# zzbuzzard/PATHS

Hardware: AMD Instinct MI355X
Metric: slides_per_sec_5level_K2048_D1024 (higher is better)
Workload: dtype f32 (products as 2 fp16 planes per operand = 22 bits, 3 fp16 MFMAs per block, fp32 accumulate); 1 GPU; 5-level PATHS recursion (forward, eval): K=2048 patches/level (level-0 grid 32x64, top_k 512, 10% background), D=1024 features, trans_dim 128 x 4 heads x 2 layers, LSTM ctx 256; 8 HBM-resident slides per GPU; slides_per_gpu=8, global_batch=8, levels=5, resident_batches_rotated=3, parallelism=slide-sharded x1 (no data-path collective)

## Files before the change

include/paths_hip.h:

```cpp
#ifndef PATHS_HIP_H
#define PATHS_HIP_H

#include <stddef.h>
#include <stdint.h>

#ifdef __cplusplus
extern "C" {
#endif

typedef void* paths_stream_t;

const char* paths_last_error(void);
const char* paths_build_info(void);
int paths_abi_version(void);

void* paths_event_create(void);
void* paths_stream_create_masked(const uint32_t* cu_mask, int words);
int paths_event_destroy(void* event);
int paths_stream_wait(paths_stream_t dst, paths_stream_t src, void* event);
int paths_set_stop_event(void* event);
int paths_flush_stop_event(paths_stream_t src);
int paths_stop_event_pending(void);
int paths_clear_stop_event(void);
int paths_record_event(void* event, paths_stream_t stream);
int paths_stream_wait_event(paths_stream_t dst, void* event);
int paths_memset_zero(void* p, size_t bytes, paths_stream_t stream);

int paths_lstm_cell(const float* x, int64_t ldx, const float* h0, int64_t ldh0, const float* c0, int64_t ldc0,
                    const float* w_gates, const float* b_gates, const float* w_mem, const float* b_mem,
                    float* state_out, int64_t ldso, float* y, int64_t ldy, float* ws_o, float* save_frm, float* save_tc,
                    const float* hp, const int* hp_row,
                    int M, int D, int Hc, const int64_t* num_ims, int rows_per_slide, int phases, paths_stream_t stream);

int paths_pe_table(const float* div_term, int pe_mode, int d, int rows, float* out, paths_stream_t stream);
int paths_importance_proj(const float* y, int64_t ldy, const float* w_ip, const float* b1, const float* w2, const float* b2 ,
                          const float* bp, const float* special, const float* div_term, const float* pe_table, int pe_rows,
                          const int64_t* locs,
                          const int64_t* num_ims, int rows_per_slide, int patch_size, int pe_mode, int imp_mul,
                          float* importance, float* tokens, float* save_hid, float* save_pproj, int M, int D, int Hi, int d,
                          int skip_padding, paths_stream_t stream);

int64_t paths_x6_packed_bytes(int Npad, int K, int planes);
int paths_x6_pack_weights(const float* w, int64_t ldw, void* out, int N, int Npad, int K, int planes, float w_scale,
                          paths_stream_t stream);
int paths_x6_pack_weights_t(const float* w, int64_t ldw, void* out, int N, int Npad, int K, int Kvalid, int planes, paths_stream_t stream);
int paths_lstm_cell_x6(const float* x, int64_t ldx, const int64_t* x_rows, const float* h0, int64_t ldh0, const float* c0, int64_t ldc0,
                       const void* w_gates_x6, const float* b_gates, const void* w_mem_x6, const float* b_mem,
                       float* state_out, int64_t ldso, float* y, int64_t ldy, float* ws_o, float* save_frm, float* save_tc,
                       const float* hp, const int* hp_row,
                       int M, int D, int Hc, const int64_t* num_ims, int rows_per_slide, int phases,
                       int planes, float wg_scale, float wm_scale, float a_scale, paths_stream_t stream);
int paths_lstm_cell_x6_h16(const float* x, int64_t ldx, const int64_t* x_rows, const float* h0, int64_t ldh0, const float* c0, int64_t ldc0,
                           const void* w_gates_x6, const float* b_gates, const void* w_mem_x6, const float* b_mem,
                           float* state_out, int64_t ldso, float* y, int64_t ldy, float* ws_o, float* save_frm, float* save_tc,
                           const float* hp, const int* hp_row,
                           int M, int D, int Hc, const int64_t* num_ims, int rows_per_slide, int phases,
                           int planes, float wg_scale, float wm_scale, float a_scale, paths_stream_t stream);
int paths_importance_proj_x6(const float* y, int64_t ldy, const int64_t* y_rows, const float* y_add, int64_t ldya, const void* w_ip_x6, const float* b1, const float* w2, const float* b2 ,
                             const float* bp, const float* special, const float* div_term, const float* pe_table, int pe_rows,
                             const int64_t* locs,
                             const int64_t* num_ims, int rows_per_slide, int patch_size, int pe_mode, int imp_mul,
                             float* importance, float* tokens, float* save_hid, float* save_pproj, int M, int D, int Hi, int d,
                             int skip_padding, int planes, float w_scale, float a_scale, float* splitk_ws, paths_stream_t stream);
int paths_importance_proj_x6_h16(const float* y, int64_t ldy, const int64_t* y_rows, const float* y_add, int64_t ldya, const void* w_ip_x6, const float* b1, const float* w2, const float* b2 ,
                                 const float* bp, const float* special, const float* div_term, const float* pe_table, int pe_rows,
                                 const int64_t* locs,
                                 const int64_t* num_ims, int rows_per_slide, int patch_size, int pe_mode, int imp_mul,
                                 float* importance, float* tokens, float* save_hid, float* save_pproj, int M, int D, int Hi, int d,
                                 int skip_padding, int planes, float w_scale, float a_scale, float* splitk_ws, paths_stream_t stream);
int64_t paths_importance_proj_x6_workspace(int M);
int paths_importance_qkv_x6(const float* y, int64_t ldy, const int64_t* y_rows, const float* y_add, int64_t ldya, const void* w_ip_x6,
                            const float* b1, const float* w2, const float* b2 , const float* bp, const float* special,
                            const float* pe_table, int pe_rows, const int64_t* locs, const int64_t* num_ims, int B, int N,
                            int patch_size, int pe_mode, int imp_mul, float* importance, float* tokens, int D, int skip_padding,
                            float w_scale, float a_scale, float* splitk_ws, const void* w_qkv, const float* bqkv, float s_wqkv,
                            float qscale, void* qkv_images, int phases, int alpha_from_importance, paths_stream_t stream);
int paths_importance_qkv_x6_h16(const float* y, int64_t ldy, const int64_t* y_rows, const float* y_add, int64_t ldya, const void* w_ip_x6,
                                const float* b1, const float* w2, const float* b2 , const float* bp, const float* special,
                                const float* pe_table, int pe_rows, const int64_t* locs, const int64_t* num_ims, int B, int N,
                                int patch_size, int pe_mode, int imp_mul, float* importance, float* tokens, int D, int skip_padding,
                                float w_scale, float a_scale, float* splitk_ws, const void* w_qkv, const float* bqkv, float s_wqkv,
                                float qscale, void* qkv_images, int phases, int alpha_from_importance, paths_stream_t stream);
int paths_gemm_nt_x6(const float* a, int64_t lda, const void* w_x6, int Kpacked, int k0, const float* b, float* out, int64_t ldo,
                     int M, int N, int Npad, int K, int act, const float* residual, int64_t ldr, const float* mask,
                     int64_t ldm, int accumulate, int planes, float w_scale, float a_scale, paths_stream_t stream);
int paths_gemm_add_nt_x6(const float* a, int64_t lda, const int64_t* a_rows, const float* a_add, int64_t ld_add, const void* w_x6, int Kpacked,
                         const float* b, float* out, int64_t ldo, int M, int N, int Npad, int K, int act, const int64_t* num_ims,
                         int rows_per_slide, float w_scale, float a_scale, paths_stream_t stream);
int paths_gemm_add_nt_x6_h16(const float* a, int64_t lda, const int64_t* a_rows, const float* a_add, int64_t ld_add, const void* w_x6, int Kpacked,
                             const float* b, float* out, int64_t ldo, int M, int N, int Npad, int K, int act, const int64_t* num_ims,
                             int rows_per_slide, float w_scale, float a_scale, paths_stream_t stream);
int paths_gemm_rows_nt_x6(const int64_t* a_rows, const void* w_x6, int Kpacked, int k0, float* out, int64_t ldo,
                          int M, int Npad, int K, int planes, float w_scale, float a_scale, paths_stream_t stream);

int paths_gemm_nt_f32(const float* a, int64_t lda, const float* w, int64_t ldw, const float* b, float* out, int64_t ldo,
                      int M, int N, int Npad, int K, int act, const float* residual, int64_t ldr, const float* mask,
                      int64_t ldm, int accumulate, paths_stream_t stream);
int64_t paths_gemm_tn_workspace(int N1, int N2, int splits);
int paths_gemm_tn_f32(const float* a, int64_t lda, const float* b0, int64_t ldb0, int nb0, const float* b1, int64_t ldb1,
                      float* out, int64_t ldo, int M, int N1, int N2, int splits, int accumulate, float* workspace,
                      paths_stream_t stream);
int paths_gemm_tn_x6(const float* a, int64_t lda, const float* b0, int64_t ldb0, int nb0, const float* b1, int64_t ldb1,
                     float* out, int64_t ldo, int M, int N1, int N2, int splits, int accumulate, float* workspace, int planes,
                     paths_stream_t stream);
int paths_colsum_f32(const float* a, int64_t lda, int M, int N, float* out, int splits, int accumulate, float* workspace,
                     paths_stream_t stream);
int paths_transpose_f32(const float* in, int64_t ldi, int R, int C, float* out, int64_t ldo, paths_stream_t stream);

int paths_adamw_chunk(void);
int paths_adamw_multi(const int64_t* table, const int64_t* numel, const int32_t* blocks, int nblocks, const float* step_size,
                      const float* bc2_sqrt, float wd_scale, int has_wd, float lerp_w, float beta2, float value, float eps, int flavor,
                      paths_stream_t stream);

int paths_lstm_bwd_a(const float* dh1, int64_t ldd, const float* dh1b, int64_t lddb, const float* o, const float* tc,
                     const int64_t* num_ims, int rows_per_slide, int64_t M, int D, float* dpre_o, int64_t ldo,
                     float* dpre_h, paths_stream_t stream);
int paths_lstm_bwd_b(const float* dc1_h, const float* dc1_ext, int64_t lde, const float* frm, const float* c0, int64_t ldc0,
                     const int64_t* num_ims, int rows_per_slide, int64_t M, int Hc, float* dg, int64_t ldg, float* dc0,
                     int64_t lddc0, paths_stream_t stream);
int paths_importance_bwd(const float* dtok, const float* pproj, const float* hid, const float* alpha, const float* w2,
                         const int64_t* num_ims, int rows_per_slide, int64_t M, int imp_mul, float* du, float* da, float* dah,
                         paths_stream_t stream);
int paths_layernorm_fwd_stats(const float* x, const float* add, const float* gamma, const float* beta, float* y, float* xhat,
                              float* rstd, int64_t rows, int d, float eps, paths_stream_t stream);
int paths_layernorm_bwd(const float* dy, const float* xhat, const float* rstd, const float* gamma, float* dx, float* dyxhat,
                        int64_t rows, int d, paths_stream_t stream);
int paths_layernorm_bwd_sums(const float* dy, const float* xhat, const float* rstd, const float* gamma, float* dx, float* slabs,
                             int64_t rows, int d, int rows_per_block, paths_stream_t stream);
int paths_reduce_slabs_f32(const float* slabs, int splits, int n, float* out, int accumulate, paths_stream_t stream);
int paths_defer_reductions(int on);
int paths_flush_reductions(int* n_entries, paths_stream_t stream);

int paths_attention_bwd_f32(const float* q, const float* k, const float* v, const float* o, const float* d_o, const float* lse,
                            const int64_t* num_ims, float* dqkv, float* ws_dsum, int B, int T, int H, int head_dim,
                            paths_stream_t stream);
int64_t paths_attention_token0_workspace(int B, int T, int H);
int paths_attention_token0_any(const float* qkv, int64_t ld, const int64_t* num_ims, float* a0, float* ws, int B, int T, int H, int head_dim,
                               float qscale, paths_stream_t stream);
int paths_attention_token0_fwd(const float* q, const float* k, const float* v, const int64_t* num_ims, float* a0, float* lse0, float* ws,
                               int B, int T, int H, int head_dim, uint64_t drop_key, float drop_p, paths_stream_t stream);
int paths_attention_token0_bwd(const float* q, const float* k, const float* v, const float* a0, const float* da0, const float* lse0,
                               const int64_t* num_ims, float* dqkv, float* ws, int B, int T, int H, int head_dim, uint64_t drop_key,
                               float drop_p, paths_stream_t stream);
int64_t paths_token0_attention_workspace(int B, int T, int d, int H);
int paths_token0_attention(const float* x, const int64_t* num_ims, const float* in_proj_weight, const float* in_proj_bias, float* attn_patch,
                           int64_t patch_ld, float* attn_self, int64_t self_ld, float* ws, int B, int T, int d, int H, int special_last,
                           paths_stream_t stream);
int64_t paths_attention_rollout_workspace(int B, int T, int d, int H);
int paths_attention_rollout_prepare(const float* x, const int64_t* num_ims, const float* in_proj_weight, const float* in_proj_bias, float* ws,
                                    int B, int T, int d, int H, int special_last, paths_stream_t stream);
int paths_attention_rollout_seed(const float* attn_patch, int64_t patch_ld, const float* attn_self, int64_t self_ld, const int64_t* num_ims,
                                 float* r, float* rollout, int64_t rollout_ld, float* rollout_self, int B, int T, int H, paths_stream_t stream);
int paths_attention_rollout_step(const float* ws, const int64_t* num_ims, const float* r_in, float* r_out, float* rollout, int64_t rollout_ld,
                                 float* rollout_self, int B, int T, int d, int H, paths_stream_t stream);

int paths_linear_f32(const float* a, int64_t lda, const float* w, const float* b, float* out, int64_t ldo,
                     int M, int N, int Npad, int K, int act, paths_stream_t stream);

int paths_attention_f32(const float* q, const float* k, const float* v, float* o, float* lse, const int64_t* num_ims,
                        int B, int T, int H, int head_dim, int max_queries, paths_stream_t stream);

int64_t paths_attention_x6_workspace(int B, int T, int H, int head_dim, int planes);
int paths_attention_x6(const float* q, const float* k, const float* v, float* o, float* lse, const int64_t* num_ims,
                       int B, int T, int H, int head_dim, int max_queries, void* workspace, int planes, int images_ready,
                       paths_stream_t stream);

int paths_token_layer_f32(const float* x_in, const float* attn, float* x_out,
                          const float* wo, const float* bo, const float* ln1g, const float* ln1b, const float* cab,
                          const float* ln2g, const float* ln2b, const float* w1, const float* b1, const float* w2,
                          const float* b2, const float* ln3g, const float* ln3b, const float* wqkv, const float* bqkv,
                          float* q, float* k, float* v, const int64_t* num_ims, int B, int T, int d, int H,
                          int do_post, int do_qkv, int skip_padding, float qscale, float eps, int max_tokens,
                          paths_stream_t stream);

int64_t paths_tlayer_h3_image_bytes(int part);
int paths_tlayer_pack_h3(int part, const float* wa, const float* wb, const float* wc, float s_a, float s_b, float s_c, void* out,
                         paths_stream_t stream);
int paths_token_layer_h3(const float* x_in, const float* attn, float* x_out, const void* w_post, const void* w_qkv,
                         const float* bo, const float* ln1g, const float* ln1b, const float* cab, const float* ln2g, const float* ln2b,
                         const float* b1, const float* b2, const float* ln3g, const float* ln3b, const float* bqkv,
                         float s_wo, float s_w1, float s_w2, float s_wqkv,
                         float* q, float* k, float* v, const int64_t* num_ims, int B, int T, int d, int H,
                         int do_post, int do_qkv, int skip_padding, float qscale, float eps, int max_tokens, void* qkv_images,
                         paths_stream_t stream);

int64_t paths_tlayer_ws_image_bytes(int part, int d);
int paths_tlayer_pack_ws(int part, const float* wa, const float* wb, const float* wc, float s_a, float s_b, float s_c, void* out, int d,
                         paths_stream_t stream);
int paths_token_layer_ws(const float* x_in, const float* attn, const void* attn_img, float* x_out, const void* w_post, const void* w_qkv,
                         const float* bo, const float* ln1g, const float* ln1b, const float* cab, const float* ln2g, const float* ln2b,
                         const float* b1, const float* b2, const float* ln3g, const float* ln3b, const float* bqkv,
                         float s_wo, float s_w1, float s_w2, float s_wqkv, void* qkv_images, const int64_t* num_ims,
                         int B, int T, int d, int H, int do_post, int do_qkv, int skip_padding, float qscale, float eps,
                         int* zero_words, int n_zero, paths_stream_t stream);
int paths_token_layer_ws_rows(const float* x_in, const float* attn, float* x_out, const void* w_post, const void* w_qkv,
                              const float* bo, const float* ln1g, const float* ln1b, const float* cab, const float* ln2g, const float* ln2b,
                              const float* b1, const float* b2, const float* ln3g, const float* ln3b, const float* bqkv,
                              float s_wo, float s_w1, float s_w2, float s_wqkv, float* qkv_rows, int64_t ld_qkv, const int64_t* num_ims,
                              int B, int T, int d, int do_post, int do_qkv, int skip_padding, float eps, paths_stream_t stream);
int paths_attention_h3_img(void* o_img, const int64_t* num_ims, int B, int T, int H, int head_dim, void* workspace, paths_stream_t stream);

int64_t paths_token0_ws_image_bytes(void);
int64_t paths_token0_ws_image_bytes_d(int d);
int64_t paths_token0_ws_partials(int B, int T);
int64_t paths_token0_ws_partials_d(int B, int T, int d);
int paths_token0_ws_supported(int B, int T, int d, int H);
int paths_token0_pack_ws(const float* wqkv, const float* bqkv, const float* wo, const float* bo, const float* w1, const float* w2, float qscale,
                         void* out, paths_stream_t stream);
int paths_token0_pack_ws_d(const float* wqkv, const float* bqkv, const float* wo, const float* bo, const float* w1, const float* w2, float qscale,
                           int d, void* out, paths_stream_t stream);
int paths_token0_tail_ws(const float* x1, const int64_t* num_ims, const void* img, const float* bv, const float* bo,
                         const float* ln1g, const float* ln1b, const float* cab, const float* ln2g, const float* ln2b,
                         const float* b1, const float* b2, const float* ln3g, const float* ln3b, const float* lnfg, const float* lnfb,
                         const float* ctx_prev, int64_t ctx_stride, const float* ctx_all, int ctx_depth,
                         const float* wcls, const float* bcls, int num_logits, int cls_in,
                         float* ctx_out, float* logits, float* partials, int* counters, int* status, int B, int T, int d, int H,
                         float eps, float eps_final, int special_last , paths_stream_t stream);

int paths_attention_any(const float* qkv, int64_t ld, float* o, const int64_t* num_ims, int B, int T, int H, int head_dim, float qscale,
                        int max_queries, paths_stream_t stream);
int64_t paths_attention_h3_any_workspace(int B, int T, int H, int head_dim);
int paths_attention_h3_any(const float* qkv, int64_t ld, float* o, const int64_t* num_ims, int B, int T, int H, int head_dim, float qscale,
                           void* workspace, paths_stream_t stream);
int paths_attention_h3_any_img(float* o, const int64_t* num_ims, int B, int T, int H, int head_dim, void* workspace, paths_stream_t stream);
int paths_layernorm_rows(const float* x, int64_t ldx, const float* add, const float* gamma, const float* beta, float* y, int64_t ldy,
                         int64_t rows, int d, float eps, paths_stream_t stream);
int paths_layernorm2_rows(const float* x, int64_t ldx, const float* g1, const float* b1, const float* add, const float* g2, const float* b2,
                          float* y, int64_t ldy, int64_t rows, int d, float eps, paths_stream_t stream);
int paths_importance_rows(const float* hid, int64_t ldh, const float* w2, const float* b2, const int64_t* num_ims, int rows_per_slide,
                          int64_t M, int Hi, float* importance, int relu , paths_stream_t stream);
int paths_tokens_assemble(const float* P, int64_t ldp, const float* importance, int imp_mul, const float* bp, const float* special,
                          const float* div_term, const int64_t* locs, int rows_per_slide, int patch_size, int pe_mode, int d, int B,
                          float* tokens, paths_stream_t stream);
int paths_importance_tokens_rows(const float* hid, int64_t ldh, const float* w2, const float* b2, const int64_t* num_ims, int rows_per_slide,
                                 int64_t M, int Hi, float* importance, int relu, int imp_mul, const float* bp, const float* special,
                                 const float* pe_table, int pe_rows, const int64_t* locs, int patch_size, int pe_mode, int d, float* tokens,
                                 paths_stream_t stream);
int paths_final_head_any(const float* x, int64_t slide_stride, const float* lng, const float* lnb, const float* ctx_prev, int64_t ctx_stride,
                         const float* ctx_all, int ctx_depth, const float* wcls, const float* bcls, int num_logits, int cls_in,
                         float* ctx_out, float* logits, int B, int d, float eps, paths_stream_t stream);

int paths_attention_any_train(const float* qkv, int64_t ld, float* o, float* lse, const int64_t* num_ims, int B, int T, int H, int head_dim,
                              float qscale, int max_queries, uint64_t drop_key, float drop_p, paths_stream_t stream);
int paths_attention_bwd_any(const float* qkv, int64_t ld, const float* o, const float* d_o, const float* lse, const int64_t* num_ims,
                            float* dqkv, float* ws_dsum, int B, int T, int H, int head_dim, float qscale, int max_queries,
                            uint64_t drop_key, float drop_p, paths_stream_t stream);
int paths_layernorm_fwd_stats_any(const float* x, const float* add, const float* gamma, const float* beta, float* y, float* xhat,
                                  float* rstd, int64_t rows, int d, float eps, paths_stream_t stream);
int paths_layernorm_bwd_any(const float* dy, const float* xhat, const float* rstd, const float* gamma, float* dx, float* dyxhat,
                            int64_t rows, int d, paths_stream_t stream);
int paths_layernorm_bwd_sums_any(const float* dy, const float* xhat, const float* rstd, const float* gamma, float* dx, float* slabs,
                                 int64_t rows, int d, int rows_per_block, paths_stream_t stream);
int paths_importance_rows_bwd_any(const float* dz_rows, const float* x, int D, const float* hid, const float* alpha, const float* w2,
                                  const int64_t* num_ims, int rows_per_slide, int64_t M, int Hi, float* dh, float* da, float* dah,
                                  paths_stream_t stream);
int paths_importance_bwd_any(const float* dtok, const float* pproj, const float* hid, const float* alpha, const float* w2,
                             const int64_t* num_ims, int rows_per_slide, int64_t M, int imp_mul, int Hi, int d, int64_t ldu, float* du,
                             float* da, float* dah, paths_stream_t stream);

int paths_token0_tail(const float* x_in, const float* q, const float* k, const float* v, const int64_t* num_ims,
                      const float* wo, const float* bo, const float* ln1g, const float* ln1b, const float* cab,
                      const float* ln2g, const float* ln2b, const float* w1, const float* b1, const float* w2,
                      const float* b2, const float* ln3g, const float* ln3b, const float* lnfg, const float* lnfb,
                      const float* ctx_prev, int64_t ctx_stride, const float* ctx_all, int ctx_depth,
                      const float* wcls, const float* bcls, int num_logits, int cls_in,
                      float* ctx_out, float* logits, float* ws_partials, int B, int T, int d, int H, float eps,
                      float eps_final, paths_stream_t stream);

int paths_final_head(const float* x, int64_t slide_stride, const float* lng, const float* lnb,
                     const float* ctx_prev, int64_t ctx_stride, const float* ctx_all, int ctx_depth,
                     const float* wcls, const float* bcls, int num_logits, int cls_in,
                     float* ctx_out, float* logits, int B, int d, float eps, paths_stream_t stream);

int paths_layernorm_f32(const float* x, const float* gamma, const float* beta, float* y, int64_t rows, int d,
                        float eps, paths_stream_t stream);

int paths_topk(const float* scores, int64_t ld, const int64_t* num_ims, int B, int n_max, int keep,
               int* keep_idx, int64_t ldk, int* keep_count, paths_stream_t stream);
int paths_topk_rows(const float* scores, int64_t ld, const int64_t* num_ims, int B, int n_max, int keep,
                    int* keep_idx, int64_t ldk, int* keep_count, const float* row_base, int64_t row_ld, int64_t slide_rows,
                    int64_t* kept_rows, const float* zero_row, paths_stream_t stream);

int paths_expand_children(const int* keep_idx, int64_t ldk, const int* keep_count, const int64_t* locs, int64_t n_cur,
                          int patch_size, const int* next_x, const int* next_y, const int64_t* mask_ptrs, int B,
                          int64_t n_next, int64_t* num_out, int64_t* locs_out, int64_t* parent_out, int* src_row,
                          int* src_cell, int* status, int* child_pos, int* hp_row, paths_stream_t stream);

int paths_candidate_children(const int* keep_idx, int64_t ldk, const int* keep_count, const int64_t* locs, int64_t n_cur,
                             int patch_size, const int* next_x, const int* next_y, int B, int* cand_count, int64_t* cand_cells,
                             int* cand_slot, paths_stream_t stream);
int paths_admit_children(const int* cand_count, const int64_t* cand_cells, const int* cand_slot, const uint8_t* cand_mask,
                         const int* keep_idx, int64_t ldk, const int* keep_count, int patch_size, int B, int64_t n_next,
                         int64_t* num_out, int64_t* locs_out, int64_t* parent_out, int* src_row, int* src_cell, int* status,
                         int* child_pos, int* hp_row, paths_stream_t stream);

int paths_fallback_all_cells(const int* next_x, const int* next_y, const int64_t* mask_ptrs, int patch_size, int B,
                             int64_t n_next, int64_t* num_out, int64_t* locs_out, int64_t* parent_out, int* src_row,
                             int* src_cell, int* status, int* hp_row, paths_stream_t stream);

int paths_gather_rows(const int64_t* grid_ptrs, const int* src_cell, int D, const float* state_cur, int64_t n_cur,
                      int64_t ld_state_cur, const int* src_row, int Dp, const int64_t* num_out, int B, int64_t n_next,
                      float* fts_out, float* state_out, int zero_pad, int64_t* row_ptrs, const float* zero_row,
                      paths_stream_t stream);
int paths_gather_rows_h16(const int64_t* grid_ptrs, const int* src_cell, int D, const float* state_cur, int64_t n_cur,
                          int64_t ld_state_cur, const int* src_row, int Dp, const int64_t* num_out, int B, int64_t n_next,
                          float* fts_out, float* state_out, int zero_pad, int64_t* row_ptrs, const float* zero_row,
                          paths_stream_t stream);

int paths_gather_kept_rows(const float* src, int64_t n_cur, int64_t ld_src, const int* keep_idx, int64_t ldk, const int* keep_count,
                           int D, int B, float* out, paths_stream_t stream);

int paths_gather_rows_bwd(const int* keep_idx, int64_t ldk, const int* keep_count, const int* child_pos, const float* d_next,
                          int64_t n_next, int Dp, float* d_cur, int64_t n_cur, int B, paths_stream_t stream);

int paths_sibling_sum(const int* keep_idx, int64_t ldk, const int* keep_count, const int* child_pos, const float* src, int64_t n_src,
                      int64_t ld_src, int width, float* dst, int64_t n_dst, int64_t ld_dst, int B, paths_stream_t stream);
int paths_scatter_kept_rows(const float* src, int64_t ldk, int64_t ld_src, const int* keep_idx, const int* keep_count, float* dst,
                            int64_t n_dst, int64_t ld_dst, int width, int B, paths_stream_t stream);

int paths_level0_batch(const int64_t* grid_ptrs, const int* gx, const int* gy, int B, int D, int patch_size, int64_t n0,
                       float* fts, int64_t* locs, int64_t* parent, int64_t* num_ims, int zero_pad, int64_t* row_ptrs,
                       const float* zero_row, paths_stream_t stream);
int paths_level0_batch_h16(const int64_t* grid_ptrs, const int* gx, const int* gy, int B, int D, int patch_size, int64_t n0,
                           float* fts, int64_t* locs, int64_t* parent, int64_t* num_ims, int zero_pad, int64_t* row_ptrs,
                           const float* zero_row, paths_stream_t stream);

int paths_stage_rows(int64_t* row_ptrs, int64_t rows, int row_bytes, void* stage, const void* zero_row, paths_stream_t stream);

int paths_saliency_rows(const float* dx, int64_t ldd, const float* x, int64_t ldx, const int64_t* num_ims, int rows_per_slide, int D,
                        int B, float* gxi, float* gnorm, paths_stream_t stream);

int paths_scale_add_rows(const float* x, const float* alpha, const float* h, const int64_t* num_ims, int rows_per_slide,
                         int D, int64_t M, int use_alpha, float* z, paths_stream_t stream);

int paths_tissue_mask(const float* grid, int64_t cells, int D, uint8_t* mask, paths_stream_t stream);

int paths_tissue_mask_absmax(const float* grid, int64_t cells, int D, uint8_t* mask, uint32_t* absmax_bits, paths_stream_t stream);
int paths_tissue_mask_absmax_h16(const void* grid, int64_t cells, int D, uint8_t* mask, uint32_t* absmax_bits, paths_stream_t stream);

int paths_synth_grid(float* grid, int X, int Y, int D, uint32_t slide_level_key, int level, uint64_t bg_threshold,
                     paths_stream_t stream);
int paths_synth_grid_h16(void* grid, int X, int Y, int D, uint32_t slide_level_key, int level, uint64_t bg_threshold,
                         paths_stream_t stream);

int paths_importance_rows_bwd(const float* dz_rows, const float* x, int D, const float* hid, const float* alpha, const float* w2,
                              const int64_t* num_ims, int rows_per_slide, int64_t M, float* dh, float* da, float* dah,
                              paths_stream_t stream);


int paths_dropout_rows(const float* x, int64_t ldx, const float* vec, const float* resid, int64_t ldr, float* out, int64_t ldo,
                       int64_t M, int N, uint64_t key, float p, paths_stream_t stream);
int paths_dropout_mask(float* mask, int64_t n, uint64_t key, float p, paths_stream_t stream);
int64_t paths_attention_fp8_workspace(int B, int T, int H, int head_dim);
int paths_attention_fp8(const float* q, const float* k, const float* v, float* o, const int64_t* num_ims, int B, int T, int H,
                        int head_dim, void* workspace, paths_stream_t stream);
int paths_attention_fp8_qkv(const float* qkv, int64_t ld, float* o, const int64_t* num_ims, int B, int T, int H, int head_dim, float qscale,
                            void* workspace, paths_stream_t stream);

int paths_fp8_scale(const float* x, int64_t ld, int64_t M, int K, float* scale, unsigned int* scratch, const int64_t* num_ims,
                    int rows_per_slide, paths_stream_t stream);
int paths_fp8_pack_weight(const float* w, int64_t ldw, int N, int K, uint8_t* w8, float* scale, unsigned int* scratch, paths_stream_t stream);
int paths_fp8_quantize(const float* x, int64_t ld, int M, int K, const float* scale, uint8_t* x8, paths_stream_t stream);
int paths_gemm_nt_fp8(const uint8_t* a8, const uint8_t* w8, const float* a_scale, const float* w_scale, const float* bias,
                      float* out, int64_t ldo, int M, int N, int K, int act, const float* residual, int64_t ldr, paths_stream_t stream);
int paths_gemm_nt_fp8_out8(const uint8_t* a8, const uint8_t* w8, const float* a_scale, const float* w_scale, const float* bias,
                           uint8_t* out8, const float* out_scale, unsigned int* out_absmax, int M, int N, int K, int act,
                           paths_stream_t stream);

int paths_attention_x6_dropout(const float* q, const float* k, const float* v, float* o, float* lse, const int64_t* num_ims, int B,
                               int T, int H, int head_dim, int max_queries, void* workspace, int planes, uint64_t drop_key,
                               float drop_p, paths_stream_t stream);
int paths_attention_bwd_f32_dropout(const float* q, const float* k, const float* v, const float* o, const float* d_o,
                                    const float* lse, const int64_t* num_ims, float* dqkv, float* ws_dsum, int B, int T, int H,
                                    int head_dim, uint64_t drop_key, float drop_p, paths_stream_t stream);
int64_t paths_attention_bwd_x6_workspace(int B, int T, int H, int head_dim);
int paths_attention_bwd_x6_dropout(const float* q, const float* k, const float* v, const float* o, const float* d_o, const float* lse,
                                   const int64_t* num_ims, float* dqkv, float* ws_dsum, void* images, int B, int T, int H, int head_dim,
                                   uint64_t drop_key, float drop_p, paths_stream_t stream);
int paths_attention_bwd_x6_planes(const float* q, const float* k, const float* v, const float* o, const float* d_o, const float* lse,
                                  const int64_t* num_ims, float* dqkv, float* ws_dsum, void* images, int B, int T, int H, int head_dim,
                                  uint64_t drop_key, float drop_p, int planes, paths_stream_t stream);

int64_t paths_attention_wide_workspace(int T, int head_dim);
int paths_attention_wide_fwd(const float* qkv, int64_t ld, float* o, float* lse, const int64_t* num_ims, int B, int T, int H, int head_dim,
                             float qscale, int max_queries, uint64_t drop_key, float drop_p, float* workspace, paths_stream_t stream);
int paths_attention_wide_bwd(const float* qkv, int64_t ld, const float* o, const float* d_o, const float* lse, const int64_t* num_ims,
                             float* dqkv, int B, int T, int H, int head_dim, float qscale, int max_queries, uint64_t drop_key, float drop_p,
                             float* workspace, paths_stream_t stream);

#ifdef __cplusplus
}
#endif
#endif
```

paths_amd/_lib.py:

```python
from __future__ import annotations

import ctypes as C
import os
from typing import Optional

import torch

_HERE = os.path.dirname(os.path.abspath(__file__))
LIB_PATH = os.environ.get("PATHS_HIP_LIB") or os.path.join(_HERE, "libpaths_hip.so")

_i64, _i32, _f32, _vp, _u32, _u64 = C.c_int64, C.c_int, C.c_float, C.c_void_p, C.c_uint32, C.c_uint64

SIGNATURES = {
    "paths_lstm_cell": [_vp, _i64, _vp, _i64, _vp, _i64, _vp, _vp, _vp, _vp, _vp, _i64, _vp, _i64, _vp, _vp, _vp, _vp, _vp,
                        _i32, _i32, _i32, _vp, _i32, _i32, _vp],
    "paths_pe_table": [_vp, _i32, _i32, _i32, _vp, _vp],
    "paths_importance_proj": [_vp, _i64, _vp, _vp, _vp, _vp, _vp, _vp, _vp, _vp, _i32, _vp, _vp, _i32, _i32, _i32, _i32,
                              _vp, _vp, _vp, _vp, _i32, _i32, _i32, _i32, _i32, _vp],
    "paths_gemm_nt_f32": [_vp, _i64, _vp, _i64, _vp, _vp, _i64, _i32, _i32, _i32, _i32, _i32, _vp, _i64, _vp, _i64, _i32, _vp],
    "paths_x6_pack_weights": [_vp, _i64, _vp, _i32, _i32, _i32, _i32, _f32, _vp],
    "paths_x6_pack_weights_t": [_vp, _i64, _vp, _i32, _i32, _i32, _i32, _i32, _vp],
    "paths_lstm_cell_x6": [_vp, _i64, _vp, _vp, _i64, _vp, _i64, _vp, _vp, _vp, _vp, _vp, _i64, _vp, _i64, _vp, _vp, _vp, _vp, _vp,
                           _i32, _i32, _i32, _vp, _i32, _i32, _i32, _f32, _f32, _f32, _vp],
    "paths_importance_proj_x6": [_vp, _i64, _vp, _vp, _i64, _vp, _vp, _vp, _vp, _vp, _vp, _vp, _vp, _i32, _vp, _vp, _i32, _i32, _i32, _i32,
                                 _vp, _vp, _vp, _vp, _i32, _i32, _i32, _i32, _i32, _i32, _f32, _f32, _vp, _vp],
    "paths_importance_qkv_x6": [_vp, _i64, _vp, _vp, _i64, _vp, _vp, _vp, _vp, _vp, _vp, _vp, _i32, _vp, _vp, _i32, _i32, _i32, _i32, _i32,
                                _vp, _vp, _i32, _i32, _f32, _f32, _vp, _vp, _vp, _f32, _f32, _vp, _i32, _i32, _vp],
    "paths_gemm_nt_x6": [_vp, _i64, _vp, _i32, _i32, _vp, _vp, _i64, _i32, _i32, _i32, _i32, _i32, _vp, _i64, _vp, _i64, _i32,
                         _i32, _f32, _f32, _vp],
    "paths_gemm_add_nt_x6": [_vp, _i64, _vp, _vp, _i64, _vp, _i32, _vp, _vp, _i64, _i32, _i32, _i32, _i32, _i32, _vp, _i32, _f32, _f32, _vp],
    "paths_gemm_tn_f32": [_vp, _i64, _vp, _i64, _i32, _vp, _i64, _vp, _i64, _i32, _i32, _i32, _i32, _i32, _vp, _vp],
    "paths_attention_fp8": [_vp, _vp, _vp, _vp, _vp, _i32, _i32, _i32, _i32, _vp, _vp],
    "paths_gemm_tn_x6": [_vp, _i64, _vp, _i64, _i32, _vp, _i64, _vp, _i64, _i32, _i32, _i32, _i32, _i32, _vp, _i32, _vp],
    "paths_colsum_f32": [_vp, _i64, _i32, _i32, _vp, _i32, _i32, _vp, _vp],
    "paths_transpose_f32": [_vp, _i64, _i32, _i32, _vp, _i64, _vp],
    "paths_attention_wide_fwd": [_vp, _i64, _vp, _vp, _vp, _i32, _i32, _i32, _i32, _f32, _i32, _u64, _f32, _vp, _vp],
    "paths_attention_wide_bwd": [_vp, _i64, _vp, _vp, _vp, _vp, _vp, _i32, _i32, _i32, _i32, _f32, _i32, _u64, _f32, _vp, _vp],
    "paths_sibling_sum": [_vp, _i64, _vp, _vp, _vp, _i64, _i64, _i32, _vp, _i64, _i64, _i32, _vp],
    "paths_scatter_kept_rows": [_vp, _i64, _i64, _vp, _vp, _vp, _i64, _i64, _i32, _i32, _vp],
    "paths_adamw_multi": [_vp, _vp, _vp, _i32, _vp, _vp, _f32, _i32, _f32, _f32, _f32, _f32, _i32, _vp],
    "paths_lstm_bwd_a": [_vp, _i64, _vp, _i64, _vp, _vp, _vp, _i32, _i64, _i32, _vp, _i64, _vp, _vp],
    "paths_lstm_bwd_b": [_vp, _vp, _i64, _vp, _vp, _i64, _vp, _i32, _i64, _i32, _vp, _i64, _vp, _i64, _vp],
    "paths_importance_bwd": [_vp, _vp, _vp, _vp, _vp, _vp, _i32, _i64, _i32, _vp, _vp, _vp, _vp],
    "paths_layernorm_fwd_stats": [_vp, _vp, _vp, _vp, _vp, _vp, _vp, _i64, _i32, _f32, _vp],
    "paths_attention_bwd_f32": [_vp, _vp, _vp, _vp, _vp, _vp, _vp, _vp, _vp, _i32, _i32, _i32, _i32, _vp],
    "paths_attention_token0_any": [_vp, _i64, _vp, _vp, _vp, _i32, _i32, _i32, _i32, _f32, _vp],
    "paths_attention_token0_fwd": [_vp, _vp, _vp, _vp, _vp, _vp, _vp, _i32, _i32, _i32, _i32, _u64, _f32, _vp],
    "paths_attention_token0_bwd": [_vp, _vp, _vp, _vp, _vp, _vp, _vp, _vp, _vp, _i32, _i32, _i32, _i32, _u64, _f32, _vp],
    "paths_token0_attention": [_vp, _vp, _vp, _vp, _vp, _i64, _vp, _i64, _vp, _i32, _i32, _i32, _i32, _i32, _vp],
    "paths_attention_rollout_prepare": [_vp, _vp, _vp, _vp, _vp, _i32, _i32, _i32, _i32, _i32, _vp],
    "paths_attention_rollout_seed": [_vp, _i64, _vp, _i64, _vp, _vp, _vp, _i64, _vp, _i32, _i32, _i32, _vp],
    "paths_attention_rollout_step": [_vp, _vp, _vp, _vp, _vp, _i64, _vp, _i32, _i32, _i32, _i32, _vp],
    "paths_layernorm_bwd": [_vp, _vp, _vp, _vp, _vp, _vp, _i64, _i32, _vp],
    "paths_layernorm_bwd_sums": [_vp, _vp, _vp, _vp, _vp, _vp, _i64, _i32, _i32, _vp],
    "paths_reduce_slabs_f32": [_vp, _i32, _i32, _vp, _i32, _vp],
    "paths_defer_reductions": [_i32],
    "paths_flush_reductions": [_vp, _vp],
    "paths_linear_f32": [_vp, _i64, _vp, _vp, _vp, _i64, _i32, _i32, _i32, _i32, _i32, _vp],
    "paths_attention_f32": [_vp, _vp, _vp, _vp, _vp, _vp, _i32, _i32, _i32, _i32, _i32, _vp],
    "paths_attention_x6": [_vp, _vp, _vp, _vp, _vp, _vp, _i32, _i32, _i32, _i32, _i32, _vp, _i32, _i32, _vp],
    "paths_tlayer_pack_h3": [_i32, _vp, _vp, _vp, _f32, _f32, _f32, _vp, _vp],
    "paths_token_layer_h3": [_vp] * 16 + [_f32, _f32, _f32, _f32, _vp, _vp, _vp, _vp, _i32, _i32, _i32, _i32, _i32, _i32, _i32, _f32, _f32, _i32, _vp, _vp],
    "paths_tlayer_pack_ws": [_i32, _vp, _vp, _vp, _f32, _f32, _f32, _vp, _i32, _vp],
    "paths_token_layer_ws": [_vp] * 17 + [_f32, _f32, _f32, _f32, _vp, _vp, _i32, _i32, _i32, _i32, _i32, _i32, _i32, _f32, _f32, _vp, _i32, _vp],
    "paths_token_layer_ws_rows": [_vp] * 16 + [_f32, _f32, _f32, _f32, _vp, _i64, _vp, _i32, _i32, _i32, _i32, _i32, _i32, _f32, _vp],
    "paths_token0_pack_ws": [_vp, _vp, _vp, _vp, _vp, _vp, _f32, _vp, _vp],
    "paths_token0_pack_ws_d": [_vp, _vp, _vp, _vp, _vp, _vp, _f32, _i32, _vp, _vp],
    "paths_token0_tail_ws": [_vp] * 16 + [_vp, _i64, _vp, _i32, _vp, _vp, _i32, _i32, _vp, _vp, _vp, _vp, _vp, _i32, _i32, _i32, _i32, _f32, _f32, _i32, _vp],
    "paths_attention_any": [_vp, _i64, _vp, _vp, _i32, _i32, _i32, _i32, _f32, _i32, _vp],
    "paths_attention_any_train": [_vp, _i64, _vp, _vp, _vp, _i32, _i32, _i32, _i32, _f32, _i32, _u64, _f32, _vp],
    "paths_layernorm_fwd_stats_any": [_vp, _vp, _vp, _vp, _vp, _vp, _vp, _i64, _i32, _f32, _vp],
    "paths_layernorm_bwd_any": [_vp, _vp, _vp, _vp, _vp, _vp, _i64, _i32, _vp],
    "paths_layernorm_bwd_sums_any": [_vp, _vp, _vp, _vp, _vp, _vp, _i64, _i32, _i32, _vp],
    "paths_importance_bwd_any": [_vp, _vp, _vp, _vp, _vp, _vp, _i32, _i64, _i32, _i32, _i32, _i64, _vp, _vp, _vp, _vp],
    "paths_importance_rows_bwd_any": [_vp, _vp, _i32, _vp, _vp, _vp, _vp, _i32, _i64, _i32, _vp, _vp, _vp, _vp],
    "paths_attention_bwd_any": [_vp, _i64, _vp, _vp, _vp, _vp, _vp, _vp, _i32, _i32, _i32, _i32, _f32, _i32, _u64, _f32, _vp],
    "paths_fp8_scale": [_vp, _i64, _i64, _i32, _vp, _vp, _vp, _i32, _vp],
    "paths_fp8_pack_weight": [_vp, _i64, _i32, _i32, _vp, _vp, _vp, _vp],
    "paths_fp8_quantize": [_vp, _i64, _i32, _i32, _vp, _vp, _vp],
    "paths_gemm_nt_fp8_out8": [_vp, _vp, _vp, _vp, _vp, _vp, _vp, _vp, _i32, _i32, _i32, _i32, _vp],
    "paths_gemm_nt_fp8": [_vp, _vp, _vp, _vp, _vp, _vp, _i64, _i32, _i32, _i32, _i32, _vp, _i64, _vp],
    "paths_attention_fp8_qkv": [_vp, _i64, _vp, _vp, _i32, _i32, _i32, _i32, _f32, _vp, _vp],
    "paths_attention_h3_any": [_vp, _i64, _vp, _vp, _i32, _i32, _i32, _i32, _f32, _vp, _vp],
    "paths_attention_h3_any_img": [_vp, _vp, _i32, _i32, _i32, _i32, _vp, _vp],
    "paths_layernorm_rows": [_vp, _i64, _vp, _vp, _vp, _vp, _i64, _i64, _i32, _f32, _vp],
    "paths_layernorm2_rows": [_vp, _i64, _vp, _vp, _vp, _vp, _vp, _vp, _i64, _i64, _i32, _f32, _vp],
    "paths_importance_rows": [_vp, _i64, _vp, _vp, _vp, _i32, _i64, _i32, _vp, _i32, _vp],
    "paths_importance_tokens_rows": [_vp, _i64, _vp, _vp, _vp, _i32, _i64, _i32, _vp, _i32, _i32, _vp, _vp, _vp, _i32, _vp, _i32, _i32, _i32, _vp, _vp],
    "paths_tokens_assemble": [_vp, _i64, _vp, _i32, _vp, _vp, _vp, _vp, _i32, _i32, _i32, _i32, _i32, _vp, _vp],
    "paths_final_head_any": [_vp, _i64, _vp, _vp, _vp, _i64, _vp, _i32, _vp, _vp, _i32, _i32, _vp, _vp, _i32, _i32, _f32, _vp],
    "paths_attention_h3_img": [_vp, _vp, _i32, _i32, _i32, _i32, _vp, _vp],
    "paths_token_layer_f32": [_vp] * 21 + [_vp, _i32, _i32, _i32, _i32, _i32, _i32, _i32, _f32, _f32, _i32, _vp],
    "paths_token0_tail": [_vp] * 20 + [_vp, _i64, _vp, _i32, _vp, _vp, _i32, _i32, _vp, _vp, _vp, _i32, _i32, _i32, _i32, _f32, _f32, _vp],
    "paths_final_head": [_vp, _i64, _vp, _vp, _vp, _i64, _vp, _i32, _vp, _vp, _i32, _i32, _vp, _vp, _i32, _i32, _f32, _vp],
    "paths_layernorm_f32": [_vp, _vp, _vp, _vp, _i64, _i32, _f32, _vp],
    "paths_topk": [_vp, _i64, _vp, _i32, _i32, _i32, _vp, _i64, _vp, _vp],
    "paths_topk_rows": [_vp, _i64, _vp, _i32, _i32, _i32, _vp, _i64, _vp, _vp, _i64, _i64, _vp, _vp, _vp],
    "paths_gemm_rows_nt_x6": [_vp, _vp, _i32, _i32, _vp, _i64, _i32, _i32, _i32, _i32, _f32, _f32, _vp],
    "paths_expand_children": [_vp, _i64, _vp, _vp, _i64, _i32, _vp, _vp, _vp, _i32, _i64, _vp, _vp, _vp, _vp, _vp, _vp, _vp, _vp, _vp],
    "paths_candidate_children": [_vp, _i64, _vp, _vp, _i64, _i32, _vp, _vp, _i32, _vp, _vp, _vp, _vp],
    "paths_admit_children": [_vp, _vp, _vp, _vp, _vp, _i64, _vp, _i32, _i32, _i64, _vp, _vp, _vp, _vp, _vp, _vp, _vp, _vp, _vp],
    "paths_gather_kept_rows": [_vp, _i64, _i64, _vp, _i64, _vp, _i32, _i32, _vp, _vp],
    "paths_gather_rows_bwd": [_vp, _i64, _vp, _vp, _vp, _i64, _i32, _vp, _i64, _i32, _vp],
    "paths_fallback_all_cells": [_vp, _vp, _vp, _i32, _i32, _i64, _vp, _vp, _vp, _vp, _vp, _vp, _vp, _vp],
    "paths_gather_rows": [_vp, _vp, _i32, _vp, _i64, _i64, _vp, _i32, _vp, _i32, _i64, _vp, _vp, _i32, _vp, _vp, _vp],
    "paths_level0_batch": [_vp, _vp, _vp, _i32, _i32, _i32, _i64, _vp, _vp, _vp, _vp, _i32, _vp, _vp, _vp],
    "paths_scale_add_rows": [_vp, _vp, _vp, _vp, _i32, _i32, _i64, _i32, _vp, _vp],
    "paths_importance_rows_bwd": [_vp, _vp, _i32, _vp, _vp, _vp, _vp, _i32, _i64, _vp, _vp, _vp, _vp],
    "paths_dropout_rows": [_vp, _i64, _vp, _vp, _i64, _vp, _i64, _i64, _i32, _u64, _f32, _vp],
    "paths_dropout_mask": [_vp, _i64, _u64, _f32, _vp],
    "paths_attention_x6_dropout": [_vp, _vp, _vp, _vp, _vp, _vp, _i32, _i32, _i32, _i32, _i32, _vp, _i32, _u64, _f32, _vp],
    "paths_attention_bwd_f32_dropout": [_vp, _vp, _vp, _vp, _vp, _vp, _vp, _vp, _vp, _i32, _i32, _i32, _i32, _u64, _f32, _vp],
    "paths_attention_bwd_x6_dropout": [_vp, _vp, _vp, _vp, _vp, _vp, _vp, _vp, _vp, _vp, _i32, _i32, _i32, _i32, _u64, _f32, _vp],
    "paths_attention_bwd_x6_planes": [_vp, _vp, _vp, _vp, _vp, _vp, _vp, _vp, _vp, _vp, _i32, _i32, _i32, _i32, _u64, _f32, _i32, _vp],
    "paths_stream_wait": [_vp, _vp, _vp],
    "paths_set_stop_event": [_vp],
    "paths_flush_stop_event": [_vp],
    "paths_stream_wait_event": [_vp, _vp],
    "paths_record_event": [_vp, _vp],
    "paths_event_destroy": [_vp],
    "paths_memset_zero": [_vp, C.c_size_t, _vp],
    "paths_tissue_mask": [_vp, _i64, _i32, _vp, _vp],
    "paths_tissue_mask_absmax": [_vp, _i64, _i32, _vp, _vp, _vp],
    "paths_synth_grid": [_vp, _i32, _i32, _i32, _u32, _i32, _u64, _vp],
    "paths_stage_rows": [_vp, _i64, _i32, _vp, _vp, _vp],
    "paths_saliency_rows": [_vp, _i64, _vp, _i64, _vp, _i32, _i32, _i32, _vp, _vp, _vp],
}
for _n in ("paths_lstm_cell_x6", "paths_importance_proj_x6", "paths_importance_qkv_x6", "paths_gemm_add_nt_x6", "paths_gather_rows",
           "paths_level0_batch", "paths_tissue_mask_absmax", "paths_synth_grid"):
    SIGNATURES[_n + "_h16"] = SIGNATURES[_n]
_PLAIN = {"paths_gemm_tn_workspace": (C.c_int64, [_i32, _i32, _i32]), "paths_x6_packed_bytes": (C.c_int64, [_i32, _i32, _i32]), "paths_tlayer_h3_image_bytes": (C.c_int64, [_i32]), "paths_tlayer_ws_image_bytes": (C.c_int64, [_i32, _i32]), "paths_token0_ws_image_bytes": (C.c_int64, []), "paths_token0_ws_partials": (C.c_int64, [_i32, _i32]), "paths_token0_ws_image_bytes_d": (C.c_int64, [_i32]), "paths_token0_ws_partials_d": (C.c_int64, [_i32, _i32, _i32]), "paths_token0_ws_supported": (_i32, [_i32, _i32, _i32, _i32]), "paths_attention_x6_workspace": (C.c_int64, [_i32, _i32, _i32, _i32, _i32]), "paths_attention_fp8_workspace": (C.c_int64, [_i32, _i32, _i32, _i32]), "paths_attention_bwd_x6_workspace": (C.c_int64, [_i32, _i32, _i32, _i32]), "paths_attention_token0_workspace": (C.c_int64, [_i32, _i32, _i32]), "paths_token0_attention_workspace": (C.c_int64, [_i32, _i32, _i32, _i32]), "paths_attention_rollout_workspace": (C.c_int64, [_i32, _i32, _i32, _i32]), "paths_attention_h3_any_workspace": (C.c_int64, [_i32, _i32, _i32, _i32]), "paths_importance_proj_x6_workspace": (C.c_int64, [_i32]), "paths_last_error": (C.c_char_p, []), "paths_build_info": (C.c_char_p, []), "paths_abi_version": (_i32, []), "paths_stop_event_pending": (_i32, []), "paths_clear_stop_event": (_i32, []), "paths_adamw_chunk": (_i32, []), "paths_attention_wide_workspace": (C.c_int64, [_i32, _i32]), "paths_event_create": (_vp, []), "paths_stream_create_masked": (_vp, [_vp, _i32])}

ABI_VERSION = 3
_lib: Optional[C.CDLL] = None


class PathsHipError(RuntimeError):
    pass


def load() -> C.CDLL:
    global _lib
    if _lib is None:
        if not os.path.isfile(LIB_PATH):
            raise PathsHipError(f"{LIB_PATH} not found: the HIP extension is not built (run __graft_entry__.build()); "
                                "paths_amd has no CPU fallback")
        lib = C.CDLL(LIB_PATH)
        lib.paths_abi_version.restype = _i32
        if lib.paths_abi_version() != ABI_VERSION:
            raise PathsHipError(f"{LIB_PATH} has ABI version {lib.paths_abi_version()}, this binding needs {ABI_VERSION}: rebuild it "
                                "(__graft_entry__.build())")
        for name, args in SIGNATURES.items():
            fn = getattr(lib, name)
            fn.argtypes, fn.restype = args, _i32
        for name, (res, args) in _PLAIN.items():
            fn = getattr(lib, name)
            fn.argtypes, fn.restype = args, res
        _lib = lib
    return _lib


def ptr(t):
    if t is None or type(t) is int:
        return t
    return t.data_ptr()


_RAW_STREAM = getattr(torch._C, "_cuda_getCurrentRawStream", None)
_GET_DEVICE = getattr(torch._C, "_cuda_getDevice", None)


def stream() -> int:
    if _RAW_STREAM is not None and _GET_DEVICE is not None:
        return _RAW_STREAM(_GET_DEVICE())
    return torch.cuda.current_stream().cuda_stream


TAPE = None
TAPE_EVENTS = None


def call(name: str, *args):
    lib = load()
    fn = getattr(lib, name)
    rc = fn(*args)
    if rc != 0:
        raise PathsHipError(f"{name} failed ({rc}): {lib.paths_last_error().decode()}")
    if TAPE is not None:
        TAPE.append((fn, args, name))
        fb = fork_behind.active
        if fb is not None and fb.taken_at is None and name != "paths_set_stop_event" and not lib.paths_stop_event_pending():
            fb.taken_at = len(TAPE) - 1


def stream_wait(dst: "torch.cuda.Stream", src: "torch.cuda.Stream"):
    dst.wait_stream(src)
    if TAPE is not None:
        lib = load()
        pool = TAPE_EVENTS if TAPE_EVENTS is not None else [[], 0]
        if pool[1] == len(pool[0]):
            ev = lib.paths_event_create()
            if not ev:
                raise PathsHipError("paths_event_create failed")
            pool[0].append(ev)
        ev = pool[0][pool[1]]
        pool[1] += 1
        TAPE.append((lib.paths_stream_wait, (dst.cuda_stream, src.cuda_stream, ev), "paths_stream_wait"))


STOP_EVENTS = __import__("os").environ.get("PATHS_STOP_EVENTS", "1") != "0"


_TAPE_PLUMBING = {"paths_set_stop_event", "paths_flush_stop_event", "paths_stream_wait_event", "paths_stream_wait", "paths_record_event",
                  "paths_clear_stop_event"}


class fork_behind:

    active = None

    def __init__(self, dsts, src):
        self.dsts, self.src = list(dsts), src
        self.ev = None
        self.taken_at = None

    def __enter__(self):
        if TAPE is not None and STOP_EVENTS:
            lib = load()
            pool = TAPE_EVENTS if TAPE_EVENTS is not None else [[], 0]
            if pool[1] == len(pool[0]):
                e = lib.paths_event_create()
                if not e:
                    raise PathsHipError("paths_event_create failed")
                pool[0].append(e)
            self.ev = pool[0][pool[1]]
            pool[1] += 1
            call("paths_set_stop_event", self.ev)
            self.prev, fork_behind.active = fork_behind.active, self
        return self

    def __exit__(self, et, ev, tb):
        if self.ev is not None:
            fork_behind.active = self.prev
            if et is not None:
                load().paths_clear_stop_event()
                return False
            call("paths_flush_stop_event", self.src.cuda_stream)
            if self.taken_at is not None and any(nm not in _TAPE_PLUMBING for _, _, nm in TAPE[self.taken_at + 1:]):
                call("paths_record_event", self.ev, self.src.cuda_stream)
            for d in self.dsts:
                call("paths_stream_wait_event", d.cuda_stream, self.ev)
        elif et is None:
            for d in self.dsts:
                stream_wait(d, self.src)
        return False


def zeros(shape, **kw) -> torch.Tensor:
    t = torch.zeros(shape, **kw)
    if TAPE is not None:
        TAPE.append((load().paths_memset_zero, (t.data_ptr(), t.numel() * t.element_size(), stream()), "paths_memset_zero"))
    return t


def require_cuda(*tensors: torch.Tensor):
    for t in tensors:
        if t is not None and not t.is_cuda:
            raise PathsHipError("paths_amd runs on the GPU only: got a CPU tensor (no CPU fallback)")


def float_from_bits(bits: int) -> float:
    import struct
    bits &= 0xFFFFFFFF
    return float("inf") if bits >= 0x7F800000 else struct.unpack("<f", struct.pack("<I", bits))[0]


def absmax(t: torch.Tensor) -> float:
    require_cuda(t)
    assert t.dtype == torch.float32 and t.is_contiguous() and t.numel() % 4 == 0
    bits = torch.zeros((1,), dtype=torch.int32, device=t.device)
    D = t.shape[-1] if (t.dim() > 1 and t.shape[-1] % 4 == 0) else 4
    call("paths_tissue_mask_absmax", t.data_ptr(), t.numel() // D, D, None, bits.data_ptr(), stream())
    return float_from_bits(int(bits.item()))
```

paths_amd/csrc/gemm_x6.hip:

```cpp
#include "common.h"
#include "gemm_epi.h"
#include "finish_qkv.h"
#include "split.h"

#ifndef PATHS_X6_PART
#define PATHS_X6_PART 0
#endif

namespace {
using namespace paths_epi;

constexpr int FRAG = 1024;
template <int NP> constexpr int planes_of() { return NP == 4 ? 2 : NP; }
template <int NP> constexpr int subt() { return planes_of<NP>() * FRAG; }

struct X6Operands {
  const float* A0; int64_t lda0; int K0;
  const int64_t* A0rows;
  const float* A1; int64_t lda1; int K1;
  const float* Aadd; int64_t ldadd;
  const char* Wt;
  int64_t w_group_stride;
  int M;
  const int64_t* num_ims;
  int rows_per_slide;
  float a_scale;
  int ksplit = 1;
};

template <int NP, int WTM, int WTN, int PF, bool ADD, bool ROWS, class Epi, int OCC = 1, bool A16 = false>
__global__ void __launch_bounds__(256) __attribute__((amdgpu_waves_per_eu(OCC, OCC)))
gemm_x6_kernel(X6Operands g, Epi epi) {
  static_assert(NP == 2 || NP == 3 || NP == 4, "two fp16 planes, three bf16 planes or two bf16 planes");
  static_assert(!A16 || (NP == 2 && ROWS), "fp16 A rows: two-plane fp16 split, row-pointer form");
  constexpr int PL = planes_of<NP>();
  constexpr bool A1P = A16 && !ADD;
  constexpr int PLA = A1P ? 1 : PL;
  constexpr int SUBT = subt<NP>();
  constexpr int SUBTA = PLA * FRAG;
  constexpr int NPROD = NP == 3 ? 6 : A1P ? 2 : 3;
  constexpr int BM = WTM * 64, BN = WTN * 64;
  constexpr int SA = 2 * WTM, SB = 2 * WTN;
  constexpr int STAGE = SA * SUBTA + SB * SUBT;
  constexpr int NA = BM / 64;
  constexpr int NPB = SB * PL, NB = (NPB + 3) / 4;
  static_assert(WTM % 2 == 0, "A fragment register slots alternate per accumulator row");
  extern __shared__ __attribute__((aligned(16))) char smem[];
  const int tid = threadIdx.x, lane = tid & 63, wave = __builtin_amdgcn_readfirstlane(tid >> 6), wm = wave >> 1, wn = wave & 1;

  const int nbx = gridDim.x, nby = gridDim.y, nblk = nbx * nby;
  const int lin = xcd_tile_order(blockIdx.y * nbx + blockIdx.x, nblk);
  constexpr int GM = 8;
  const int per_group = GM * nbx;
  const int grp = lin / per_group, in_grp = lin - grp * per_group;
  const int rows_in_grp = min(GM, nby - grp * GM);
  const int by = grp * GM + in_grp % rows_in_grp, bx = in_grp / rows_in_grp;
  const int m0 = by * BM, n0 = bx * BN;
  if (block_all_padding(g.num_ims, g.rows_per_slide, m0, BM, g.M)) return;

  const int arow = tid >> 2, ac = tid & 3;
  uint32_t aoff0[NA], aoff1[NA], aoffs[ADD ? NA : 1]; int awr[NA];
  typedef const f32x4 __attribute__((address_space(1))) * gptr_f4;
  typedef const u32x2 __attribute__((address_space(1))) * gptr_h4;
  gptr_f4 rowp[ROWS && !A16 ? NA : 1];
  gptr_h4 rowh[A16 ? NA : 1];
#pragma unroll
  for (int p = 0; p < NA; ++p) {
    const int row = p * 64 + arow;
    const int64_t grow = min(m0 + row, g.M - 1);
    aoff0[p] = ROWS ? 0u : (uint32_t)((grow * g.lda0 + 4 * ac) * 4);
    if constexpr (A16) rowh[p] = reinterpret_cast<gptr_h4>(static_cast<uintptr_t>(g.A0rows[grow]) + 8 * ac);
    else if constexpr (ROWS) rowp[p] = reinterpret_cast<gptr_f4>(static_cast<uintptr_t>(g.A0rows[grow]) + 16 * ac);
    aoff1[p] = (uint32_t)((grow * g.lda1 + 4 * ac) * 4);
    if constexpr (ADD) aoffs[p] = (uint32_t)((grow * g.ldadd + 4 * ac) * 4);
    awr[p] = (row >> 5) * SUBTA + (ac >> 1) * 512 + (row & 31) * 16 + (ac & 1) * 8;
  }
  const int K0w = g.ksplit > 1 ? g.K0 / g.ksplit : g.K0;
  const int kofs = g.ksplit > 1 ? (int)blockIdx.z * K0w : 0;
  if (kofs != 0) {
#pragma unroll
    for (int p = 0; p < NA; ++p) {
      aoff0[p] += (uint32_t)kofs * 4u;
      if constexpr (A16) rowh[p] += kofs >> 2;
      else if constexpr (ROWS) rowp[p] += kofs >> 2;
      if constexpr (ADD) aoffs[p] += (uint32_t)kofs * 4u;
    }
  }
  const int nk0 = K0w >> 4, nk = (K0w + g.K1) >> 4;
  const char* bbase[NB]; int bwr[NB];
#pragma unroll
  for (int i = 0; i < NB; ++i) {
    int pc = wave + 4 * i;
    if (pc >= NPB) pc -= 4;
    const int sub = pc / PL, pl = pc % PL;
    bbase[i] = g.Wt + ((int64_t)(n0 >> 5) + sub) * g.w_group_stride + pl * FRAG;
    bwr[i] = (A1P ? SA * SUBTA + sub * SUBT : (SA + sub) * SUBT) + pl * FRAG + lane * 16;
  }
  static_assert(PF == 1 || PF == 2, "one or two register sets");
  f32x4 sa[PF][NA], sadd[ADD ? PF : 1][ADD ? NA : 1]; u32x4 sbr[PF][NB];
  u32x2 sh[A16 ? PF : 1][A16 ? NA : 1];
  uint32_t hi[NA][2], mid[NP != 2 ? NA : 1][2], lo[NA][2];
  float* const anyA = const_cast<float*>(ROWS ? reinterpret_cast<const float*>(g.Wt) : g.A0);
  const auto rsA0 = __builtin_amdgcn_make_buffer_rsrc(anyA, 0, 0xFFFFFFFFu, 0x00020000);
  const auto rsA1 = __builtin_amdgcn_make_buffer_rsrc(g.A1 ? const_cast<float*>(g.A1) : anyA, 0, 0xFFFFFFFFu, 0x00020000);
  const auto rsAdd = __builtin_amdgcn_make_buffer_rsrc(ADD ? const_cast<float*>(g.Aadd) : anyA, 0, 0xFFFFFFFFu, 0x00020000);
  const auto rsW = __builtin_amdgcn_make_buffer_rsrc(const_cast<char*>(g.Wt), 0, 0xFFFFFFFFu, 0x00020000);
  const int lane16 = lane * 16;
  int bsoff[NB];
#pragma unroll
  for (int i = 0; i < NB; ++i) bsoff[i] = (int)(bbase[i] - g.Wt) + (kofs >> 4) * SUBT;
  auto gload_a = [&](int set, int q, int kt) {
    const bool first = kt < nk0;
    const int soff = (first ? kt : kt - nk0) * 64;
    if constexpr (A16) {
      sh[set][q] = rowh[q][kt * 4];
    } else if constexpr (ROWS) {
      sa[set][q] = rowp[q][kt * 4];
    } else {
      const u32x4 raw = first ? __builtin_amdgcn_raw_buffer_load_b128(rsA0, (int)aoff0[q], soff, 0)
                              : __builtin_amdgcn_raw_buffer_load_b128(rsA1, (int)aoff1[q], soff, 0);
      sa[set][q] = __builtin_bit_cast(f32x4, raw);
    }
    if constexpr (ADD) {
      sadd[set][q] = __builtin_bit_cast(f32x4, __builtin_amdgcn_raw_buffer_load_b128(rsAdd, (int)aoffs[q], kt * 64, 0));
    }
  };
  auto gload_b = [&](int set, int q, int kt) {
    sbr[set][q] = __builtin_amdgcn_raw_buffer_load_b128(rsW, lane16, bsoff[q] + kt * SUBT, 0);
  };
  constexpr int PRE = ADD ? (A16 ? 2 : 1) : 0;
  constexpr int NS = A1P ? 2 : (NP == 3 ? 12 : NP == 4 ? 7 : 5) + PRE;
  float tf[NA][2];
  const uint32_t s2 = A1P ? __builtin_bit_cast(uint32_t, f16x2{(_Float16)g.a_scale, (_Float16)g.a_scale}) : 0u;
  auto a_step = [&](int set, int q, int st0, int buf) __attribute__((always_inline)) {
    f32x4& v = sa[set][q];
    const int st = st0 - PRE;
    if constexpr (ADD && A16) {
      if (st0 == 0) { v[0] = h_lo(sh[set][q][0]) + sadd[set][q][0]; v[1] = h_hi(sh[set][q][0]) + sadd[set][q][1]; }
      if (st0 == 1) { v[2] = h_lo(sh[set][q][1]) + sadd[set][q][2]; v[3] = h_hi(sh[set][q][1]) + sadd[set][q][3]; }
    } else if constexpr (ADD) {
      if (st0 == 0) v += sadd[set][q];
    }
    if constexpr (A1P) {
      if (st == 0) {
        asm("v_pk_mul_f16 %0, %1, %2" : "=v"(hi[q][0]) : "v"(sh[set][q][0]), "v"(s2));
        asm("v_pk_mul_f16 %0, %1, %2" : "=v"(hi[q][1]) : "v"(sh[set][q][1]), "v"(s2));
      }
      if (st == 1) *reinterpret_cast<u32x2*>(smem + buf * STAGE + awr[q]) = u32x2{hi[q][0], hi[q][1]};
    } else if constexpr (NP == 3) {
      if (st == 0) { hi[q][0] = pk_bf16(v[0], v[1]); hi[q][1] = pk_bf16(v[2], v[3]); }
      if (st == 1) { tf[q][0] = bf_lo(hi[q][0]); tf[q][1] = bf_hi(hi[q][0]); }
      if (st == 2) { v[0] -= tf[q][0]; v[1] -= tf[q][1]; }
      if (st == 3) { tf[q][0] = bf_lo(hi[q][1]); tf[q][1] = bf_hi(hi[q][1]); }
      if (st == 4) { v[2] -= tf[q][0]; v[3] -= tf[q][1]; }
      if (st == 5) { mid[q][0] = pk_bf16(v[0], v[1]); mid[q][1] = pk_bf16(v[2], v[3]); }
      if (st == 6) { tf[q][0] = bf_lo(mid[q][0]); tf[q][1] = bf_hi(mid[q][0]); }
      if (st == 7) { v[0] -= tf[q][0]; v[1] -= tf[q][1]; }
      if (st == 8) { tf[q][0] = bf_lo(mid[q][1]); tf[q][1] = bf_hi(mid[q][1]); }
      if (st == 9) { v[2] -= tf[q][0]; v[3] -= tf[q][1]; }
      if (st == 10) { lo[q][0] = pk_bf16(v[0], v[1]); lo[q][1] = pk_bf16(v[2], v[3]); }
      if (st == 11) {
        char* d = smem + buf * STAGE + awr[q];
        *reinterpret_cast<u32x2*>(d) = u32x2{hi[q][0], hi[q][1]};
        *reinterpret_cast<u32x2*>(d + FRAG) = u32x2{mid[q][0], mid[q][1]};
        *reinterpret_cast<u32x2*>(d + 2 * FRAG) = u32x2{lo[q][0], lo[q][1]};
      }
    } else if constexpr (NP == 4) {
      if (st == 0) { hi[q][0] = pk_bf16(v[0], v[1]); hi[q][1] = pk_bf16(v[2], v[3]); }
      if (st == 1) { tf[q][0] = bf_lo(hi[q][0]); tf[q][1] = bf_hi(hi[q][0]); }
      if (st == 2) { v[0] -= tf[q][0]; v[1] -= tf[q][1]; }
      if (st == 3) { tf[q][0] = bf_lo(hi[q][1]); tf[q][1] = bf_hi(hi[q][1]); }
      if (st == 4) { v[2] -= tf[q][0]; v[3] -= tf[q][1]; }
      if (st == 5) { mid[q][0] = pk_bf16(v[0], v[1]); mid[q][1] = pk_bf16(v[2], v[3]); }
      if (st == 6) {
        char* d = smem + buf * STAGE + awr[q];
        *reinterpret_cast<u32x2*>(d) = u32x2{hi[q][0], hi[q][1]};
        *reinterpret_cast<u32x2*>(d + FRAG) = u32x2{mid[q][0], mid[q][1]};
      }
    } else {
      if (st == 0) v *= g.a_scale;
      if (st == 1) { hi[q][0] = pk_f16(v[0], v[1]); hi[q][1] = pk_f16(v[2], v[3]); }
      if (st == 2) {
        asm("v_fma_mixlo_f16 %0, %1, -1.0, %2 op_sel_hi:[1,0,0]" : "=v"(lo[q][0]) : "v"(hi[q][0]), "v"(v[0]));
        asm("v_fma_mixlo_f16 %0, %1, -1.0, %2 op_sel_hi:[1,0,0]" : "=v"(lo[q][1]) : "v"(hi[q][1]), "v"(v[2]));
      }
      if (st == 3) {
        asm("v_fma_mixhi_f16 %0, %1, -1.0, %2 op_sel:[1,0,0] op_sel_hi:[1,0,0]" : "+v"(lo[q][0]) : "v"(hi[q][0]), "v"(v[1]));
        asm("v_fma_mixhi_f16 %0, %1, -1.0, %2 op_sel:[1,0,0] op_sel_hi:[1,0,0]" : "+v"(lo[q][1]) : "v"(hi[q][1]), "v"(v[3]));
      }
      if (st == 4) {
        char* d = smem + buf * STAGE + awr[q];
        *reinterpret_cast<u32x2*>(d) = u32x2{hi[q][0], hi[q][1]};
        *reinterpret_cast<u32x2*>(d + FRAG) = u32x2{lo[q][0], lo[q][1]};
      }
    }
  };
  auto swrite_b = [&](int set, int q, int buf) { *reinterpret_cast<u32x4*>(smem + buf * STAGE + bwr[q]) = sbr[set][q]; };

  f32x16 acc[WTM][WTN];
  epi.template init<WTM, WTN>(acc, m0 + wm * WTM * 32, n0 + wn * WTN * 32, lane, g.M);

  const char* sA = smem + (wm * WTM) * SUBTA + lane * 16;
  const char* sB = A1P ? smem + SA * SUBTA + (wn * WTN) * SUBT + lane * 16 : smem + (SA + wn * WTN) * SUBT + lane * 16;
  u32x4 fa[2][PLA], fb[2][WTN][PL];
  auto read_a = [&](int buf, int i, int slot, int p) { fa[slot][p] = *reinterpret_cast<const u32x4*>(sA + buf * STAGE + i * SUBTA + p * FRAG); };
  auto read_b = [&](int buf, int j, int slot, int p) { fb[slot][j][p] = *reinterpret_cast<const u32x4*>(sB + buf * STAGE + j * SUBT + p * FRAG); };
  constexpr int RG = WTN * NPROD;
  auto one_mfma = [&](int gq, int sb) __attribute__((always_inline)) {
    const int i = gq / RG, j = (gq % RG) / NPROD, t = gq % NPROD, sl = i & 1;
    if constexpr (NP == 3) {
      constexpr int PA_[6] = {2, 0, 1, 1, 0, 0}, PB_[6] = {0, 2, 1, 0, 1, 0};
      acc[i][j] = __builtin_amdgcn_mfma_f32_32x32x16_bf16(__builtin_bit_cast(bf16x8, fa[sl][PA_[t]]), __builtin_bit_cast(bf16x8, fb[sb][j][PB_[t]]), acc[i][j], 0, 0, 0);
    } else if constexpr (NP == 4) {
      constexpr int PA_[3] = {1, 0, 0}, PB_[3] = {0, 1, 0};
      acc[i][j] = __builtin_amdgcn_mfma_f32_32x32x16_bf16(__builtin_bit_cast(bf16x8, fa[sl][PA_[t]]), __builtin_bit_cast(bf16x8, fb[sb][j][PB_[t]]), acc[i][j], 0, 0, 0);
    } else if constexpr (A1P) {
      constexpr int PB_[2] = {1, 0};
      acc[i][j] = __builtin_amdgcn_mfma_f32_32x32x16_f16(__builtin_bit_cast(f16x8, fa[sl][0]), __builtin_bit_cast(f16x8, fb[sb][j][PB_[t]]), acc[i][j], 0, 0, 0);
    } else {
      constexpr int PA_[3] = {1, 0, 0}, PB_[3] = {0, 1, 0};
      acc[i][j] = __builtin_amdgcn_mfma_f32_32x32x16_f16(__builtin_bit_cast(f16x8, fa[sl][PA_[t]]), __builtin_bit_cast(f16x8, fb[sb][j][PB_[t]]), acc[i][j], 0, 0, 0);
    }
  };
  constexpr int AG = (WTM - 1) * RG;
  constexpr auto fits = [](int spg) constexpr {
    return PF == 1 ? ((NS + spg - 1) / spg) * NA + NB <= AG : (NS * NA + spg - 1) / spg + NB <= AG;
  };
  constexpr int SPG = fits(1) ? 1 : fits(2) ? 2 : fits(3) ? 3 : 4;
  static_assert(fits(SPG), "staging does not fit before the barrier");
  constexpr int GPC = (NS + SPG - 1) / SPG;
  constexpr int GA2 = (NS * NA + SPG - 1) / SPG;
  constexpr int TS = PF == 1 ? GPC * NA + NB : GA2 + NB + NA + NB;
  static_assert(TS <= WTM * RG, "staging does not fit in a stage");
  constexpr int AR0 = RG / 2;
  auto staging_slot = [&](auto sc, int kt, auto bufc, auto m1c, auto m2c) __attribute__((always_inline)) {
    constexpr int s = decltype(sc)::value, buf = decltype(bufc)::value;
    constexpr bool more1 = decltype(m1c)::value, more2 = decltype(m2c)::value;
    constexpr int set = PF == 2 ? (buf ^ 1) : 0;
    if constexpr (PF == 1) {
      if constexpr (s < GPC * NA) {
        constexpr int q = s / GPC, g0 = s % GPC;
        if constexpr (more1) {
          static_for<g0 * SPG, (g0 + 1) * SPG < NS ? (g0 + 1) * SPG : NS>([&](auto mc) __attribute__((always_inline)) {
            a_step(set, q, decltype(mc)::value, buf ^ 1);
          });
        }
        if constexpr (more2 && g0 == GPC - 1) gload_a(set, q, kt + 1 + PF);
      } else if constexpr (s < TS) {
        if constexpr (more1) swrite_b(set, s - GPC * NA, buf ^ 1);
        if constexpr (more2) gload_b(set, s - GPC * NA, kt + 1 + PF);
      }
    } else {
      if constexpr (s < GA2) {
        if constexpr (more1) {
          static_for<s * SPG, (s + 1) * SPG < NS * NA ? (s + 1) * SPG : NS * NA>([&](auto mc) __attribute__((always_inline)) {
            constexpr int m = decltype(mc)::value;
            a_step(set, m / NS, m % NS, buf ^ 1);
          });
        }
      } else if constexpr (s < GA2 + NB) {
        if constexpr (more1) swrite_b(set, s - GA2, buf ^ 1);
      } else if constexpr (s < GA2 + NB + NA) {
        if constexpr (more2) gload_a(set, s - GA2 - NB, kt + 1 + PF);
      } else if constexpr (s < TS) {
        if constexpr (more2) gload_b(set, s - GA2 - NB - NA, kt + 1 + PF);
      }
    }
  };
  auto stage_body = [&](int kt, auto bufc, auto m1c, auto m2c) __attribute__((always_inline)) {
    constexpr int buf = decltype(bufc)::value, sb = buf;
    constexpr bool more1 = decltype(m1c)::value, more2 = decltype(m2c)::value;
    constexpr int set = PF == 2 ? (buf ^ 1) : 0;
    static_for<0, AG>([&](auto gc) __attribute__((always_inline)) {
      constexpr int gq = decltype(gc)::value, i = gq / RG, gr = gq % RG;
      one_mfma(gq, sb);
      if constexpr (gr >= AR0 && gr < AR0 + PLA) read_a(buf, i + 1, (i + 1) & 1, gr - AR0);
      staging_slot(std::integral_constant<int, gq>{}, kt, bufc, m1c, m2c);
      __builtin_amdgcn_sched_barrier(0);
    });
    __syncthreads();
    __builtin_amdgcn_sched_barrier(0);
    static_for<AG, WTM * RG>([&](auto gc) __attribute__((always_inline)) {
      constexpr int gq = decltype(gc)::value, gr = gq % RG;
      one_mfma(gq, sb);
      if constexpr (more1) {
        static_for<2 * gr, 2 * gr + 2>([&](auto fc) __attribute__((always_inline)) {
          constexpr int f = decltype(fc)::value;
          if constexpr (f < PLA) read_a(buf ^ 1, 0, 0, f);
          else if constexpr (f < PLA + PL * WTN) read_b(buf ^ 1, (f - PLA) / PL, sb ^ 1, (f - PLA) % PL);
        });
      }
      staging_slot(std::integral_constant<int, gq>{}, kt, bufc, m1c, m2c);
      __builtin_amdgcn_sched_barrier(0);
    });
  };
  constexpr std::integral_constant<int, 0> I0{};
  constexpr std::integral_constant<int, 1> I1{};
  constexpr std::true_type T{};
  constexpr std::false_type F{};

#pragma unroll
  for (int q = 0; q < NA; ++q) gload_a(0, q, 0);
#pragma unroll
  for (int q = 0; q < NB; ++q) gload_b(0, q, 0);
#pragma unroll
  for (int q = 0; q < NA; ++q)
#pragma unroll
    for (int st = 0; st < NS; ++st) a_step(0, q, st, 0);
#pragma unroll
  for (int q = 0; q < NB; ++q) swrite_b(0, q, 0);
#pragma unroll
  for (int sidx = 1; sidx <= PF; ++sidx) {
#pragma unroll
    for (int q = 0; q < NA; ++q) gload_a(PF == 2 ? (sidx & 1) : 0, q, sidx);
#pragma unroll
    for (int q = 0; q < NB; ++q) gload_b(PF == 2 ? (sidx & 1) : 0, q, sidx);
  }
  __syncthreads();
#pragma unroll
  for (int p = 0; p < PLA; ++p) read_a(0, 0, 0, p);
#pragma unroll
  for (int j = 0; j < WTN; ++j)
#pragma unroll
    for (int p = 0; p < PL; ++p) read_b(0, j, 0, p);
  for (int kt = 0; kt < nk - 2 * PF; kt += 2) {
    __builtin_amdgcn_sched_barrier(0);
    stage_body(kt, I0, T, T);
    stage_body(kt + 1, I1, T, T);
  }
  if constexpr (PF == 2) {
    stage_body(nk - 4, I0, T, T);
    stage_body(nk - 3, I1, T, F);
  }
  stage_body(nk - 2, I0, T, F);
  stage_body(nk - 1, I1, F, F);
  __syncthreads();
  epi.template run<WTM, WTN, 2, 2>(acc, m0 + wm * WTM * 32, n0 + wn * WTN * 32, lane, wm, wn, g.M, reinterpret_cast<float*>(smem));
}

template <int NP>
__global__ void x6_pack_kernel(const float* __restrict__ w, int64_t ldw, uint16_t* __restrict__ out, int N, int Npad, int K, float wscale) {
  const int64_t i = blockIdx.x * (int64_t)blockDim.x + threadIdx.x;
  if (i >= (int64_t)Npad * K) return;
  const int n = (int)(i / K), k = (int)(i % K);
  const float v = n < N ? w[(int64_t)n * ldw + k] * wscale : 0.f;
  uint16_t* o = out + ((int64_t)(n >> 5) * (K >> 4) + (k >> 4)) * (subt<NP>() / 2) + ((k >> 3) & 1) * 256 + (n & 31) * 8 + (k & 7);
  if constexpr (NP == 3) {
    const __bf16 h = (__bf16)v; const float r1 = v - (float)h;
    const __bf16 m = (__bf16)r1; const float r2 = r1 - (float)m;
    const __bf16 l = (__bf16)r2;
    o[0] = __builtin_bit_cast(uint16_t, h); o[FRAG / 2] = __builtin_bit_cast(uint16_t, m); o[FRAG] = __builtin_bit_cast(uint16_t, l);
  } else if constexpr (NP == 4) {
    const __bf16 h = (__bf16)v; const float r1 = v - (float)h;
    const __bf16 m = (__bf16)r1;
    o[0] = __builtin_bit_cast(uint16_t, h); o[FRAG / 2] = __builtin_bit_cast(uint16_t, m);
  } else {
    const _Float16 h = (_Float16)v; const float r1 = v - (float)h;
    const _Float16 l = (_Float16)r1;
    o[0] = __builtin_bit_cast(uint16_t, h); o[FRAG / 2] = __builtin_bit_cast(uint16_t, l);
  }
}

template <int NP>
__global__ void x6_pack_t_kernel(const float* __restrict__ w, int64_t ldw, uint16_t* __restrict__ out, int N, int Npad, int K, int Kvalid) {
  static_assert(NP == 3 || NP == 4, "bf16 planes (scale 1)");
  const int64_t i = blockIdx.x * (int64_t)blockDim.x + threadIdx.x;
  if (i >= (int64_t)Npad * (K >> 3)) return;
  const int n = (int)(i % Npad), k0 = (int)(i / Npad) * 8;
  uint16_t h[8], m[8], l[8];
#pragma unroll
  for (int j = 0; j < 8; ++j) {
    const int k = k0 + j;
    const float v = (n < N && k < Kvalid) ? w[(int64_t)k * ldw + n] : 0.f;
    const __bf16 hh = (__bf16)v; const float r1 = v - (float)hh;
    const __bf16 mm = (__bf16)r1; const float r2 = r1 - (float)mm;
    const __bf16 ll = (__bf16)r2;
    h[j] = __builtin_bit_cast(uint16_t, hh); m[j] = __builtin_bit_cast(uint16_t, mm); l[j] = __builtin_bit_cast(uint16_t, ll);
  }
  uint16_t* o = out + ((int64_t)(n >> 5) * (K >> 4) + (k0 >> 4)) * (subt<NP>() / 2) + ((k0 >> 3) & 1) * 256 + (n & 31) * 8;
  typedef uint16_t u16x8 __attribute__((ext_vector_type(8)));
  *reinterpret_cast<u16x8*>(o) = u16x8{h[0], h[1], h[2], h[3], h[4], h[5], h[6], h[7]};
  *reinterpret_cast<u16x8*>(o + FRAG / 2) = u16x8{m[0], m[1], m[2], m[3], m[4], m[5], m[6], m[7]};
  if constexpr (NP == 3) *reinterpret_cast<u16x8*>(o + FRAG) = u16x8{l[0], l[1], l[2], l[3], l[4], l[5], l[6], l[7]};
}

template <int NP, int WTM, int WTN, int PF, bool ADD, bool ROWS, class Epi, int OCC = 1, bool A16 = false>
int launch_x6_np(const X6Operands& g, int Npad, const Epi& epi, hipStream_t stream, const char* name) {
  constexpr int BM = WTM * 64, BN = WTN * 64;
  constexpr size_t lds = 2ull * (2 * WTM * ((A16 && !ADD) ? FRAG : subt<NP>()) + 2 * WTN * subt<NP>());
  const int K = g.K0 + g.K1;
  PATHS_REQUIRE(g.M > 0, "%s: M must be > 0", name);
  PATHS_REQUIRE(g.K0 > 0 && g.K0 % 16 == 0 && g.K1 % 16 == 0 && K % 32 == 0 && K >= 128, "%s: K panels (%d,%d): multiples of 16, total a multiple of 32, >= 128", name, g.K0, g.K1);
  PATHS_REQUIRE(Npad % BN == 0, "%s: packed N (%d) must be a multiple of %d", name, Npad, BN);
  PATHS_REQUIRE(g.lda0 % 4 == 0 && g.lda1 % 4 == 0, "%s: leading dims must be multiples of 4 floats", name);
  PATHS_REQUIRE(((uintptr_t)g.A0 % 16 == 0) && ((uintptr_t)g.A1 % 16 == 0) && ((uintptr_t)g.Wt % 16 == 0), "%s: operands must be 16-byte aligned", name);
  PATHS_REQUIRE(ROWS == (g.A0rows != nullptr) && (!ROWS || g.K1 == 0), "%s: row-pointer form is single-panel", name);
  PATHS_REQUIRE((int64_t)g.M * (g.lda0 > g.lda1 ? (g.lda0 > g.ldadd ? g.lda0 : g.ldadd) : (g.lda1 > g.ldadd ? g.lda1 : g.ldadd)) * 4 < (int64_t)1 << 32, "%s: A panel larger than 4 GiB", name);
  auto kern = gemm_x6_kernel<NP, WTM, WTN, PF, ADD, ROWS, Epi, OCC, A16>;
  PATHS_LDS_OPT_IN(kern, lds, name);
  PATHS_REQUIRE(g.ksplit == 1 || (g.ksplit > 1 && g.K1 == 0 && g.K0 % (32 * g.ksplit) == 0 && g.K0 / g.ksplit >= 128), "%s: split-K needs a single panel and k windows that are multiples of 32, >= 128", name);
  dim3 grid(Npad / BN, (g.M + BM - 1) / BM, g.ksplit);
  hipLaunchKernelGGL(kern, grid, dim3(256), lds, stream, g, epi);
  PATHS_LAUNCH_CHECK(name);
  return PATHS_OK;
}

struct EpiRaw {
  float* ws; int64_t zstride; int ntn;
  template <int WTM, int WTN>
  __device__ __forceinline__ void init(f32x16 (&acc)[WTM][WTN], int, int, int, int) const {
#pragma unroll
    for (int i = 0; i < WTM; ++i)
#pragma unroll
      for (int j = 0; j < WTN; ++j)
#pragma unroll
        for (int r = 0; r < 16; ++r) acc[i][j][r] = 0.f;
  }
  template <int WTM, int WTN, int WGM, int WGN>
  __device__ __forceinline__ void run(f32x16 (&acc)[WTM][WTN], int row0, int col0, int lane, int, int, int, float*) const {
    float* base = ws + (int64_t)blockIdx.z * zstride;
#pragma unroll
    for (int i = 0; i < WTM; ++i)
#pragma unroll
      for (int j = 0; j < WTN; ++j) {
        f32x4* t = reinterpret_cast<f32x4*>(base + ((int64_t)((row0 >> 5) + i) * ntn + (col0 >> 5) + j) * 1024) + lane;
#pragma unroll
        for (int q = 0; q < 4; ++q) {
          const f32x4 v = f32x4{acc[i][j][4 * q], acc[i][j][4 * q + 1], acc[i][j][4 * q + 2], acc[i][j][4 * q + 3]};
          t[64 * q] = v;
        }
      }
  }
};

template <int NZ, class Epi>
__global__ void __launch_bounds__(256)
x6_finish_kernel(const float* __restrict__ ws, int64_t zstride, int ntn, int M, const int64_t* __restrict__ num_ims, int rows_per_slide, Epi epi) {
  extern __shared__ __attribute__((aligned(16))) char smem[];
  const int tid = threadIdx.x, lane = tid & 63, wave = __builtin_amdgcn_readfirstlane(tid >> 6), wm = wave >> 1, wn = wave & 1;
  const int m0 = blockIdx.x * 64;
  if (block_all_padding(num_ims, rows_per_slide, m0, 64, M)) return;
  const int row0 = m0 + wm * 32, col0 = wn * 128;
  f32x16 acc[1][4];
#pragma unroll
  for (int j = 0; j < 4; ++j) {
    const f32x4* t = reinterpret_cast<const f32x4*>(ws + ((int64_t)(row0 >> 5) * ntn + (col0 >> 5) + j) * 1024) + lane;
#pragma unroll
    for (int q = 0; q < 4; ++q) {
      f32x4 v = t[64 * q];
#pragma unroll
      for (int z = 1; z < NZ; ++z) v += *reinterpret_cast<const f32x4*>(reinterpret_cast<const float*>(t + 64 * q) + z * zstride);
      acc[0][j][4 * q] = v[0]; acc[0][j][4 * q + 1] = v[1]; acc[0][j][4 * q + 2] = v[2]; acc[0][j][4 * q + 3] = v[3];
    }
  }
  epi.template run<1, 4, 2, 2>(acc, row0, col0, lane, wm, wn, M, reinterpret_cast<float*>(smem));
}

template <int WTM, int WTN, int PF, bool ADD, class Epi>
int launch_x6(int planes, const X6Operands& g, int Npad, const Epi& epi, hipStream_t stream, const char* name) {
  if (g.A0rows != nullptr) {
    if (planes == 2) return launch_x6_np<2, WTM, WTN, PF, ADD, true>(g, Npad, epi, stream, name);
    return paths_set_error(PATHS_EUNSUPPORTED, "%s: row pointers need planes = 2", name);
  }
  if constexpr (std::is_same<Epi, EpiBias>::value && !ADD) {
    if (planes == 4) return launch_x6_np<4, WTM, WTN, PF, ADD, false>(g, Npad, epi, stream, name);
  }
  if (planes == 3) return launch_x6_np<3, WTM, WTN, PF, ADD, false>(g, Npad, epi, stream, name);
  if (planes == 2) return launch_x6_np<2, WTM, WTN, PF, ADD, false>(g, Npad, epi, stream, name);
  return paths_set_error(PATHS_EINVAL, "%s: planes must be 3 (bf16 x6) or 2 (fp16 x3), got %d", name, planes);
}

constexpr int H_OCC = 3;
constexpr int H_TRAIN_OCC = 2;

inline int plane_count(int planes) { return planes == 4 ? 2 : planes; }
inline int64_t group_stride(int planes, int Kpacked) { return (int64_t)(Kpacked / 16) * plane_count(planes) * FRAG; }
inline bool pow2(float x) { int e; return x > 0.f && frexpf(x, &e) == 0.5f; }
inline bool h16_scale_ok(float a_scale) { return pow2(a_scale) && a_scale >= 1.0f && a_scale <= 32768.0f; }

}

extern "C" {

#if PATHS_X6_PART == 0 || PATHS_X6_PART == 1
int64_t paths_x6_packed_bytes(int Npad, int K, int planes) { return (int64_t)Npad * K * 2 * plane_count(planes); }

int paths_x6_pack_weights(const float* w, int64_t ldw, void* out, int N, int Npad, int K, int planes, float w_scale, hipStream_t stream) {
  PATHS_REQUIRE(N > 0 && Npad >= N && Npad % 32 == 0 && K % 16 == 0, "x6_pack_weights: bad shape N=%d Npad=%d K=%d", N, Npad, K);
  PATHS_REQUIRE((uintptr_t)out % 16 == 0, "x6_pack_weights: out must be 16-byte aligned");
  PATHS_REQUIRE(((planes == 3 || planes == 4) && w_scale == 1.0f) || (planes == 2 && pow2(w_scale)), "x6_pack_weights: planes 3 / 4 (bf16) with w_scale 1, or planes 2 with a power-of-two w_scale");
  const int64_t n = (int64_t)Npad * K;
  const dim3 grid((unsigned)((n + 255) / 256));
  if (planes == 4) hipLaunchKernelGGL(x6_pack_kernel<4>, grid, dim3(256), 0, stream, w, ldw, reinterpret_cast<uint16_t*>(out), N, Npad, K, 1.0f);
  else if (planes == 3) hipLaunchKernelGGL(x6_pack_kernel<3>, grid, dim3(256), 0, stream, w, ldw, reinterpret_cast<uint16_t*>(out), N, Npad, K, 1.0f);
  else hipLaunchKernelGGL(x6_pack_kernel<2>, grid, dim3(256), 0, stream, w, ldw, reinterpret_cast<uint16_t*>(out), N, Npad, K, w_scale);
  PATHS_LAUNCH_CHECK("x6_pack_weights");
  return PATHS_OK;
}

int paths_x6_pack_weights_t(const float* w, int64_t ldw, void* out, int N, int Npad, int K, int Kvalid, int planes, hipStream_t stream) {
  PATHS_REQUIRE(N > 0 && Npad >= N && Npad % 32 == 0 && K % 16 == 0 && Kvalid > 0 && Kvalid <= K, "x6_pack_weights_t: bad shape N=%d Npad=%d K=%d Kvalid=%d", N, Npad, K, Kvalid);
  PATHS_REQUIRE(w != nullptr && out != nullptr && (uintptr_t)out % 16 == 0, "x6_pack_weights_t: null / unaligned operand");
  PATHS_REQUIRE(planes == 3 || planes == 4, "x6_pack_weights_t: planes 3 or 4 (bf16)");
  const int64_t n = (int64_t)Npad * (K / 8);
  const dim3 grid((unsigned)((n + 255) / 256));
  if (planes == 4) hipLaunchKernelGGL(x6_pack_t_kernel<4>, grid, dim3(256), 0, stream, w, ldw, reinterpret_cast<uint16_t*>(out), N, Npad, K, Kvalid);
  else hipLaunchKernelGGL(x6_pack_t_kernel<3>, grid, dim3(256), 0, stream, w, ldw, reinterpret_cast<uint16_t*>(out), N, Npad, K, Kvalid);
  PATHS_LAUNCH_CHECK("x6_pack_weights_t");
  return PATHS_OK;
}

}
namespace {
template <bool A16>
int lstm_cell_x6(const float* x, int64_t ldx, const int64_t* x_rows, const float* h0, int64_t ldh0, const float* c0, int64_t ldc0,
                 const void* w_gates_x6, const float* b_gates, const void* w_mem_x6, const float* b_mem,
                 float* state_out, int64_t ldso, float* y, int64_t ldy, float* ws_o, float* save_frm, float* save_tc,
                 const float* hp, const int* hp_row, int M, int D, int Hc, const int64_t* num_ims, int rows_per_slide,
                 int phases, int planes, float wg_scale, float wm_scale, float a_scale, hipStream_t stream) {
  PATHS_REQUIRE(D % 256 == 0 && Hc % 64 == 0, "lstm_cell_x6: D (%d) must be a multiple of 256 and Hc (%d) of 64", D, Hc);
  if constexpr (A16) {
    PATHS_REQUIRE(x_rows != nullptr && x == nullptr && planes == 2, "lstm_cell_x6_h16: fp16 rows are given as x_rows (planes = 2)");
    PATHS_REQUIRE(h16_scale_ok(a_scale), "lstm_cell_x6_h16: a_scale must be a power of two in [1, 2^15]");
  }
  PATHS_REQUIRE(hp != nullptr || (h0 == nullptr) == (c0 == nullptr), "lstm_cell_x6: h0 and c0 must both be given or both be null");
  PATHS_REQUIRE((hp == nullptr) == (hp_row == nullptr) && (hp == nullptr || h0 == nullptr),
                "lstm_cell_x6: hp/hp_row come together and replace h0 (the h half of the gate GEMM was done per parent)");
  PATHS_REQUIRE(planes == 3 || (pow2(wg_scale) && pow2(wm_scale) && pow2(a_scale)), "lstm_cell_x6: scales must be powers of two");
  PATHS_REQUIRE(x_rows == nullptr || (h0 == nullptr && y == nullptr && save_tc == nullptr), "lstm_cell_x6: x_rows (rows addressed in place) excludes h0, y and the training saves");
  if (planes == 3) wg_scale = wm_scale = a_scale = 1.0f;
  const char* wg = reinterpret_cast<const char*>(w_gates_x6);
  const int64_t gs = group_stride(planes, 2 * D);
  const float sg = 1.0f / (wg_scale * a_scale), sm = 1.0f / (wm_scale * a_scale);
  X6Operands g{x, ldx, D, x_rows, h0, h0 ? ldh0 : 0, h0 ? D : 0, nullptr, 0, wg, gs, M, num_ims, rows_per_slide, a_scale};
  const bool small_m = planes == 2 && M <= 8192 && (h0 == nullptr);
  if (phases & 1) {
    EpiLstmC e{b_gates, c0, ldc0, state_out + D, ldso, save_frm, (int64_t)3 * Hc, hp, (int64_t)3 * Hc + D, hp_row, sg};
    int rc;
    if constexpr (A16) {
      rc = small_m ? launch_x6_np<2, 2, 3, 2, false, true, decltype(e), 1, true>(g, 3 * Hc, e, stream, "lstm_cell_x6_h16(c, 128-row tiles)")
                   : launch_x6_np<2, 4, 3, 1, false, true, decltype(e), 1, true>(g, 3 * Hc, e, stream, "lstm_cell_x6_h16(c)");
    } else if (small_m) rc = x_rows ? launch_x6_np<2, 2, 3, 2, false, true>(g, 3 * Hc, e, stream, "lstm_cell_x6(c, 128-row tiles)")
                             : launch_x6_np<2, 2, 3, 2, false, false>(g, 3 * Hc, e, stream, "lstm_cell_x6(c, 128-row tiles)");
    else rc = launch_x6<4, 3, 1, false>(planes, g, 3 * Hc, e, stream, "lstm_cell_x6(c)");
    if (rc) return rc;
  }
  const bool o_raw = y == nullptr && save_tc == nullptr && save_frm == nullptr;
  if (phases & 2) {
    X6Operands go = g;
    go.Wt = wg + (int64_t)(3 * Hc / 32) * gs;
    int rc;
    if (o_raw) {
      EpiLstmORaw e{b_gates + 3 * Hc, ws_o, D, D, hp, (int64_t)3 * Hc + D, hp_row, 3 * Hc, sg};
      if constexpr (A16) {
        rc = small_m ? launch_x6_np<2, 2, 4, 2, false, true, decltype(e), 1, true>(go, D, e, stream, "lstm_cell_x6_h16(o, raw, 128-row tiles)")
                     : launch_x6_np<2, 4, 4, 1, false, true, decltype(e), 1, true>(go, D, e, stream, "lstm_cell_x6_h16(o, raw)");
      } else if (small_m) rc = x_rows ? launch_x6_np<2, 2, 4, 2, false, true>(go, D, e, stream, "lstm_cell_x6(o, raw, 128-row tiles)")
                               : launch_x6_np<2, 2, 4, 2, false, false>(go, D, e, stream, "lstm_cell_x6(o, raw, 128-row tiles)");
      else rc = launch_x6<4, 4, 1, false>(planes, go, D, e, stream, "lstm_cell_x6(o, raw)");
    } else {
      EpiLstmO e{b_gates + 3 * Hc, ws_o, D, D, hp, (int64_t)3 * Hc + D, hp_row, 3 * Hc, sg};
      if constexpr (A16) rc = launch_x6_np<2, 4, 4, 1, false, true, decltype(e), 1, true>(go, D, e, stream, "lstm_cell_x6_h16(o)");
      else rc = launch_x6<4, 4, 1, false>(planes, go, D, e, stream, "lstm_cell_x6(o)");
    }
    if (rc) return rc;
  }
  if (phases & 4) {
    X6Operands gh{state_out + D, ldso, Hc, nullptr, nullptr, 0, 0, nullptr, 0, reinterpret_cast<const char*>(w_mem_x6), group_stride(planes, Hc), M, num_ims, rows_per_slide, a_scale};
    int rc;
    PATHS_REQUIRE(save_tc == nullptr || y != nullptr, "lstm_cell_x6: save_tc (training) needs y");
    PATHS_REQUIRE(planes == 2 || planes == 3, "lstm_cell_x6: planes must be 3 (bf16 x6) or 2 (fp16 x3), got %d", planes);
    if (save_tc != nullptr) {
      EpiLstmH<true, true> e{b_mem, ws_o, D, x, ldx, state_out, ldso, y, ldy, D, save_tc, sm};
      if (planes == 2) rc = launch_x6_np<2, 2, 2, 2, false, false, decltype(e), H_TRAIN_OCC>(gh, D, e, stream, "lstm_cell_x6(h, save, 128x128)");
      else rc = launch_x6_np<3, 4, 4, 1, false, false>(gh, D, e, stream, "lstm_cell_x6(h, save)");
    } else if (y != nullptr) {
      EpiLstmH<true, false> e{b_mem, ws_o, D, x, ldx, state_out, ldso, y, ldy, D, nullptr, sm};
      rc = launch_x6<4, 4, 1, false>(planes, gh, D, e, stream, "lstm_cell_x6(h)");
    } else if (o_raw) {
      EpiLstmH<false, false, true> e{b_mem, ws_o, D, x, ldx, state_out, ldso, nullptr, 0, D, nullptr, sm};
      if (planes == 2) rc = launch_x6_np<2, 2, 2, 2, false, false, decltype(e), H_OCC>(gh, D, e, stream, "lstm_cell_x6(h, raw o, 128x128)");
      else rc = launch_x6_np<3, 4, 4, 1, false, false>(gh, D, e, stream, "lstm_cell_x6(h, raw o)");
    } else {
      EpiLstmH<false, false> e{b_mem, ws_o, D, x, ldx, state_out, ldso, nullptr, 0, D, nullptr, sm};
      if (planes == 2) rc = launch_x6_np<2, 2, 2, 2, false, false, decltype(e), H_OCC>(gh, D, e, stream, "lstm_cell_x6(h, no y, 128x128)");
      else rc = launch_x6_np<3, 4, 4, 1, false, false>(gh, D, e, stream, "lstm_cell_x6(h, no y)");
    }
    if (rc) return rc;
  }
  return PATHS_OK;
}
}
extern "C" {

int paths_lstm_cell_x6(const float* x, int64_t ldx, const int64_t* x_rows, const float* h0, int64_t ldh0, const float* c0, int64_t ldc0,
                       const void* w_gates_x6, const float* b_gates, const void* w_mem_x6, const float* b_mem,
                       float* state_out, int64_t ldso, float* y, int64_t ldy, float* ws_o, float* save_frm, float* save_tc,
                       const float* hp, const int* hp_row, int M, int D, int Hc, const int64_t* num_ims, int rows_per_slide,
                       int phases, int planes, float wg_scale, float wm_scale, float a_scale, hipStream_t stream) {
  return lstm_cell_x6<false>(x, ldx, x_rows, h0, ldh0, c0, ldc0, w_gates_x6, b_gates, w_mem_x6, b_mem, state_out, ldso, y, ldy, ws_o, save_frm,
                             save_tc, hp, hp_row, M, D, Hc, num_ims, rows_per_slide, phases, planes, wg_scale, wm_scale, a_scale, stream);
}

int paths_lstm_cell_x6_h16(const float* x, int64_t ldx, const int64_t* x_rows, const float* h0, int64_t ldh0, const float* c0, int64_t ldc0,
                           const void* w_gates_x6, const float* b_gates, const void* w_mem_x6, const float* b_mem,
                           float* state_out, int64_t ldso, float* y, int64_t ldy, float* ws_o, float* save_frm, float* save_tc,
                           const float* hp, const int* hp_row, int M, int D, int Hc, const int64_t* num_ims, int rows_per_slide,
                           int phases, int planes, float wg_scale, float wm_scale, float a_scale, hipStream_t stream) {
  return lstm_cell_x6<true>(x, ldx, x_rows, h0, ldh0, c0, ldc0, w_gates_x6, b_gates, w_mem_x6, b_mem, state_out, ldso, y, ldy, ws_o, save_frm,
                            save_tc, hp, hp_row, M, D, Hc, num_ims, rows_per_slide, phases, planes, wg_scale, wm_scale, a_scale, stream);
}

#endif
#if PATHS_X6_PART == 0 || PATHS_X6_PART == 2
int64_t paths_importance_proj_x6_workspace(int M) { return 2ll * ((M + 127) / 128 * 4) * 8 * 1024 * 4; }

}
namespace {
template <bool A16>
int importance_proj_x6(const float* y, int64_t ldy, const int64_t* y_rows, const float* y_add, int64_t ldya, const void* w_ip_x6, const float* b1, const float* w2, const float* b2,
                       const float* bp, const float* special, const float* div_term, const float* pe_table, int pe_rows, const int64_t* locs,
                       const int64_t* num_ims, int rows_per_slide, int patch_size, int pe_mode, int imp_mul,
                       float* importance, float* tokens, float* save_hid, float* save_pproj, int M, int D, int Hi, int d,
                       int skip_padding, int planes, float w_scale, float a_scale, float* splitk_ws, hipStream_t stream) {
  if constexpr (A16) {
    PATHS_REQUIRE(y == nullptr && y_rows != nullptr && y_add != nullptr && splitk_ws != nullptr && planes == 2 && D % 64 == 0 && D >= 256,
                  "importance_proj_x6_h16: fp16 rows (y_rows) + y_add on the split-K form (splitk_ws, planes = 2, D %% 64 == 0, D >= 256)");
  }
  PATHS_REQUIRE(Hi == 128 && d == 128, "importance_proj_x6: this build supports importance_mlp_hidden_dim=128, trans_dim=128 (got %d, %d)", Hi, d);
  PATHS_REQUIRE(pe_mode == 1 || pe_mode == 2, "importance_proj_x6: pe_mode must be 1 (1d) or 2 (2d)");
  PATHS_REQUIRE(pe_mode == 1 || locs != nullptr, "importance_proj_x6: 2d positional encoding needs locs");
  PATHS_REQUIRE(num_ims != nullptr && rows_per_slide > 0 && M % rows_per_slide == 0, "importance_proj_x6: bad slide layout");
  PATHS_REQUIRE(b1 != nullptr && w2 != nullptr && b2 != nullptr, "importance_proj_x6: b1, w2 and b2 (device scalar) are required");
  PATHS_REQUIRE(y_add == nullptr || (ldya % 4 == 0 && (uintptr_t)y_add % 16 == 0), "importance_proj_x6: y_add must be 16-byte aligned with ldya %% 4 == 0");
  PATHS_REQUIRE(planes == 3 || (pow2(w_scale) && pow2(a_scale)), "importance_proj_x6: scales must be powers of two");
  if (planes == 3) w_scale = a_scale = 1.0f;
  const float sc = 1.0f / (w_scale * a_scale);
  X6Operands g{y, ldy, D, y_rows, nullptr, 0, 0, y_add, ldya, reinterpret_cast<const char*>(w_ip_x6), group_stride(planes, D), M, skip_padding ? num_ims : nullptr, rows_per_slide, a_scale};
  PATHS_REQUIRE((save_hid == nullptr) == (save_pproj == nullptr), "importance_proj_x6: save_hid and save_pproj come together");
  PATHS_REQUIRE(pe_table == nullptr || pe_rows > 0, "importance_proj_x6: pe_rows must be > 0 with a pe_table");
  auto go = [&](auto epi) {
    decltype(epi) e{b1, w2, b2, bp, special, div_term, locs, num_ims, rows_per_slide, patch_size, pe_mode, imp_mul, importance, tokens,
                    save_hid, save_pproj, pe_table, pe_table ? pe_rows : 0, sc};
    {
      if (splitk_ws != nullptr && planes == 2 && (y_add != nullptr || y_rows == nullptr) && D % 64 == 0 && D >= 256) {
        const int mt = (M + 127) / 128 * 4;
        const int64_t zstride = (int64_t)mt * 8 * 1024;
        int rc;
        if constexpr (A16) {
          X6Operands gs = g; gs.ksplit = 2;
          EpiRaw raw{splitk_ws, zstride, 8};
          rc = launch_x6_np<2, 2, 4, 2, true, true, EpiRaw, 1, true>(gs, 256, raw, stream, "importance_proj_x6_h16(split-k)");
        } else {
          X6Operands gs = g; gs.ksplit = 2;
          EpiRaw raw{splitk_ws, zstride, 8};
          rc = y_add == nullptr ? launch_x6_np<2, 2, 4, 2, false, false>(gs, 256, raw, stream, "importance_proj_x6(split-k, stored y)")
               : y_rows ? launch_x6_np<2, 2, 4, 2, true, true>(gs, 256, raw, stream, "importance_proj_x6(split-k)")
                        : launch_x6_np<2, 2, 4, 2, true, false>(gs, 256, raw, stream, "importance_proj_x6(split-k)");
        }
        if (rc != PATHS_OK) return rc;
        const int fblk = (M + 63) / 64, fdepth = (fblk + 255) / 256;
        const int flds = fdepth == 1 ? 84 * 1024 : fdepth == 2 ? 54 * 1024 : fdepth == 3 ? 41 * 1024 : 1024;
        PATHS_LDS_OPT_IN((x6_finish_kernel<2, decltype(epi)>), 84 * 1024, "importance_proj_x6(finish)");
        PATHS_LAUNCH_STOP((x6_finish_kernel<2, decltype(epi)>), dim3(fblk), dim3(256), flds, stream, splitk_ws, zstride, 8, M,
                          skip_padding ? num_ims : nullptr, rows_per_slide, e);
        PATHS_LAUNCH_CHECK("importance_proj_x6(finish)");
        return PATHS_OK;
      }
    }
    if constexpr (A16) {
      return paths_set_error(PATHS_EUNSUPPORTED, "importance_proj_x6_h16: split-K form only");
    } else {
      if (y_add != nullptr) return launch_x6<2, 4, 2, true>(planes, g, 256, e, stream, "importance_proj_x6(sum)");
      return launch_x6<2, 4, 2, false>(planes, g, 256, e, stream, "importance_proj_x6");
    }
  };
  if (pe_table != nullptr) return save_hid ? go(EpiImpProj<true, true>{}) : go(EpiImpProj<true, false>{});
  return save_hid ? go(EpiImpProj<false, true>{}) : go(EpiImpProj<false, false>{});
}
}
extern "C" {

int paths_importance_proj_x6(const float* y, int64_t ldy, const int64_t* y_rows, const float* y_add, int64_t ldya, const void* w_ip_x6, const float* b1, const float* w2, const float* b2,
                             const float* bp, const float* special, const float* div_term, const float* pe_table, int pe_rows, const int64_t* locs,
                             const int64_t* num_ims, int rows_per_slide, int patch_size, int pe_mode, int imp_mul,
                             float* importance, float* tokens, float* save_hid, float* save_pproj, int M, int D, int Hi, int d,
                             int skip_padding, int planes, float w_scale, float a_scale, float* splitk_ws, hipStream_t stream) {
  return importance_proj_x6<false>(y, ldy, y_rows, y_add, ldya, w_ip_x6, b1, w2, b2, bp, special, div_term, pe_table, pe_rows, locs, num_ims,
                                   rows_per_slide, patch_size, pe_mode, imp_mul, importance, tokens, save_hid, save_pproj, M, D, Hi, d,
                                   skip_padding, planes, w_scale, a_scale, splitk_ws, stream);
}

int paths_importance_proj_x6_h16(const float* y, int64_t ldy, const int64_t* y_rows, const float* y_add, int64_t ldya, const void* w_ip_x6, const float* b1, const float* w2, const float* b2,
                                 const float* bp, const float* special, const float* div_term, const float* pe_table, int pe_rows, const int64_t* locs,
                                 const int64_t* num_ims, int rows_per_slide, int patch_size, int pe_mode, int imp_mul,
                                 float* importance, float* tokens, float* save_hid, float* save_pproj, int M, int D, int Hi, int d,
                                 int skip_padding, int planes, float w_scale, float a_scale, float* splitk_ws, hipStream_t stream) {
  return importance_proj_x6<true>(y, ldy, y_rows, y_add, ldya, w_ip_x6, b1, w2, b2, bp, special, div_term, pe_table, pe_rows, locs, num_ims,
                                  rows_per_slide, patch_size, pe_mode, imp_mul, importance, tokens, save_hid, save_pproj, M, D, Hi, d,
                                  skip_padding, planes, w_scale, a_scale, splitk_ws, stream);
}


}
namespace {
template <bool A16>
int importance_qkv_x6(const float* y, int64_t ldy, const int64_t* y_rows, const float* y_add, int64_t ldya, const void* w_ip_x6,
                      const float* b1, const float* w2, const float* b2, const float* bp, const float* special,
                      const float* pe_table, int pe_rows, const int64_t* locs, const int64_t* num_ims, int B, int N,
                      int patch_size, int pe_mode, int imp_mul, float* importance, float* tokens, int D, int skip_padding,
                      float w_scale, float a_scale, float* splitk_ws, const void* w_qkv, const float* bqkv, float s_wqkv,
                      float qscale, void* qkv_images, int phases, int alpha_from_importance, hipStream_t stream) {
  PATHS_REQUIRE(!A16 || (phases & 1) == 0 || (y == nullptr && y_rows != nullptr), "importance_qkv_x6_h16: fp16 rows are given as y_rows");
  PATHS_REQUIRE(B > 0 && N > 0 && N % 64 == 0 && D % 64 == 0 && D >= 256, "importance_qkv_x6: bad shape B=%d N=%d (a multiple of 64) D=%d", B, N, D);
  PATHS_REQUIRE(pe_mode == 1 || pe_mode == 2, "importance_qkv_x6: pe_mode must be 1 (1d) or 2 (2d)");
  PATHS_REQUIRE(pe_table != nullptr && pe_rows > 0 && (pe_mode == 1 || locs != nullptr), "importance_qkv_x6: needs the positional-encoding table (and locs in 2d mode)");
  PATHS_REQUIRE(num_ims != nullptr && splitk_ws != nullptr && (uintptr_t)splitk_ws % 16 == 0, "importance_qkv_x6: num_ims and a 16-byte aligned workspace are required");
  PATHS_REQUIRE(phases > 0 && (phases & ~7) == 0, "importance_qkv_x6: phases is a mask of 1 (GEMM), 2 (importance finish), 4 (tokens + in_proj finish)");
  PATHS_REQUIRE(pow2(w_scale) && pow2(a_scale), "importance_qkv_x6: scales must be powers of two");
  const int64_t M64 = (int64_t)B * N;
  PATHS_REQUIRE(M64 < (1ll << 24), "importance_qkv_x6: B * N must stay below 2^24 rows");
  const int M = (int)M64, T = N + 1, Tp = (T + 63) / 64 * 64;
  const int mt = (M + 127) / 128 * 4;
  const int64_t zstride = (int64_t)mt * 8 * 1024;
  if (phases & 1) {
    PATHS_REQUIRE(w_ip_x6 != nullptr && y_add != nullptr && (y != nullptr) != (y_rows != nullptr), "importance_qkv_x6: the GEMM takes (y or y_rows) + y_add");
    PATHS_REQUIRE(ldya % 4 == 0 && (uintptr_t)y_add % 16 == 0, "importance_qkv_x6: y_add must be 16-byte aligned with ldya %% 4 == 0");
    X6Operands g{y, ldy, D, y_rows, nullptr, 0, 0, y_add, ldya, reinterpret_cast<const char*>(w_ip_x6), group_stride(2, D), M, skip_padding ? num_ims : nullptr, N, a_scale};
    g.ksplit = 2;
    EpiRaw raw{splitk_ws, zstride, 8};
    int rc;
    if constexpr (A16) rc = launch_x6_np<2, 2, 4, 2, true, true, EpiRaw, 1, true>(g, 256, raw, stream, "importance_qkv_x6_h16(split-k)");
    else rc = y_rows ? launch_x6_np<2, 2, 4, 2, true, true>(g, 256, raw, stream, "importance_qkv_x6(split-k)")
                     : launch_x6_np<2, 2, 4, 2, true, false>(g, 256, raw, stream, "importance_qkv_x6(split-k)");
    if (rc != PATHS_OK) return rc;
  }
  if (phases & 6) {
    PATHS_REQUIRE(b1 && w2 && b2 && importance, "importance_qkv_x6: b1, w2, b2 (device scalar) and importance are required");
    FinQkvParams f{splitk_ws, zstride, 2, b1, w2, b2, bp, special, pe_table, pe_rows, locs, num_ims, N, T, Tp, B, patch_size, pe_mode, imp_mul,
                   skip_padding, 1.0f / (w_scale * a_scale), alpha_from_importance, importance, tokens, w_qkv, bqkv, 1.0f / s_wqkv, qscale, qkv_images,
                   (B % 8 == 0 && (M / 128) % 8 == 0 && M % 128 == 0) ? 1 : 0};
    if (phases & 2) {
      const int rc = paths_launch_finish_importance(f, stream);
      if (rc != PATHS_OK) return rc;
    }
    if (phases & 4) {
      PATHS_REQUIRE(bp && special && tokens && w_qkv && bqkv && qkv_images && pow2(s_wqkv), "importance_qkv_x6: null operand (tokens + in_proj finish)");
      PATHS_REQUIRE(((uintptr_t)tokens | (uintptr_t)w_qkv | (uintptr_t)qkv_images) % 16 == 0, "importance_qkv_x6: buffers must be 16-byte aligned");
      return paths_launch_finish_qkv(f, stream);
    }
  }
  return PATHS_OK;
}
}
extern "C" {

int paths_importance_qkv_x6(const float* y, int64_t ldy, const int64_t* y_rows, const float* y_add, int64_t ldya, const void* w_ip_x6,
                            const float* b1, const float* w2, const float* b2, const float* bp, const float* special,
                            const float* pe_table, int pe_rows, const int64_t* locs, const int64_t* num_ims, int B, int N,
                            int patch_size, int pe_mode, int imp_mul, float* importance, float* tokens, int D, int skip_padding,
                            float w_scale, float a_scale, float* splitk_ws, const void* w_qkv, const float* bqkv, float s_wqkv,
                            float qscale, void* qkv_images, int phases, int alpha_from_importance, hipStream_t stream) {
  return importance_qkv_x6<false>(y, ldy, y_rows, y_add, ldya, w_ip_x6, b1, w2, b2, bp, special, pe_table, pe_rows, locs, num_ims, B, N, patch_size,
                                  pe_mode, imp_mul, importance, tokens, D, skip_padding, w_scale, a_scale, splitk_ws, w_qkv, bqkv, s_wqkv, qscale,
                                  qkv_images, phases, alpha_from_importance, stream);
}

int paths_importance_qkv_x6_h16(const float* y, int64_t ldy, const int64_t* y_rows, const float* y_add, int64_t ldya, const void* w_ip_x6,
                                const float* b1, const float* w2, const float* b2, const float* bp, const float* special,
                                const float* pe_table, int pe_rows, const int64_t* locs, const int64_t* num_ims, int B, int N,
                                int patch_size, int pe_mode, int imp_mul, float* importance, float* tokens, int D, int skip_padding,
                                float w_scale, float a_scale, float* splitk_ws, const void* w_qkv, const float* bqkv, float s_wqkv,
                                float qscale, void* qkv_images, int phases, int alpha_from_importance, hipStream_t stream) {
  return importance_qkv_x6<true>(y, ldy, y_rows, y_add, ldya, w_ip_x6, b1, w2, b2, bp, special, pe_table, pe_rows, locs, num_ims, B, N, patch_size,
                                 pe_mode, imp_mul, importance, tokens, D, skip_padding, w_scale, a_scale, splitk_ws, w_qkv, bqkv, s_wqkv, qscale,
                                 qkv_images, phases, alpha_from_importance, stream);
}

#endif
#if PATHS_X6_PART == 0 || PATHS_X6_PART == 3
int paths_gemm_nt_x6(const float* a, int64_t lda, const void* w_x6, int Kpacked, int k0, const float* b, float* out, int64_t ldo,
                     int M, int N, int Npad, int K, int act, const float* residual, int64_t ldr, const float* mask,
                     int64_t ldm, int accumulate, int planes, float w_scale, float a_scale, hipStream_t stream) {
  PATHS_REQUIRE(k0 % 16 == 0 && k0 >= 0 && k0 + K <= Kpacked, "gemm_nt_x6: bad k window");
  PATHS_REQUIRE(planes == 3 || planes == 4 || (planes == 2 && pow2(w_scale) && pow2(a_scale)), "gemm_nt_x6: planes 3 / 4 (bf16), or planes 2 with power-of-two scales");
  if (planes != 2) w_scale = a_scale = 1.0f;
  X6Operands g{a, lda, K, nullptr, nullptr, 0, 0, nullptr, 0, reinterpret_cast<const char*>(w_x6) + (int64_t)(k0 / 16) * plane_count(planes) * FRAG, group_stride(planes, Kpacked), M, nullptr, 0, a_scale};
  EpiBias e{b, out, ldo, N, act, residual, ldr, mask, ldm, accumulate, 1.0f / (w_scale * a_scale)};
  if (Npad % 256 != 0) {
    if (planes == 4) return launch_x6_np<4, 2, 2, 2, false, false, EpiBias, 2>(g, Npad, e, stream, "gemm_nt_x6(n128, bf16 x 2)");
    if (planes == 3) return launch_x6_np<3, 2, 2, 2, false, false, EpiBias, 2>(g, Npad, e, stream, "gemm_nt_x6(n128)");
    return launch_x6_np<2, 2, 2, 2, false, false, EpiBias, 2>(g, Npad, e, stream, "gemm_nt_x6(n128)");
  }
  return launch_x6<2, 4, 2, false>(planes, g, Npad, e, stream, "gemm_nt_x6");
}

int paths_gemm_rows_nt_x6(const int64_t* a_rows, const void* w_x6, int Kpacked, int k0, float* out, int64_t ldo,
                          int M, int Npad, int K, int planes, float w_scale, float a_scale, hipStream_t stream) {
  PATHS_REQUIRE(a_rows != nullptr && planes == 2 && pow2(w_scale) && pow2(a_scale), "gemm_rows_nt_x6: row addresses need planes = 2 with power-of-two scales");
  PATHS_REQUIRE(k0 % 16 == 0 && k0 >= 0 && k0 + K <= Kpacked, "gemm_rows_nt_x6: bad k window");
  X6Operands g{nullptr, K, K, a_rows, nullptr, 0, 0, nullptr, 0,
               reinterpret_cast<const char*>(w_x6) + (int64_t)(k0 / 16) * planes * FRAG, group_stride(planes, Kpacked), M, nullptr, 0, a_scale};
  EpiBias e{nullptr, out, ldo, Npad, 0, nullptr, 0, nullptr, 0, 0, 1.0f / (w_scale * a_scale)};
  return launch_x6<2, 4, 2, false>(planes, g, Npad, e, stream, "gemm_rows_nt_x6");
}

int paths_gemm_add_nt_x6(const float* a, int64_t lda, const int64_t* a_rows, const float* a_add, int64_t ld_add, const void* w_x6, int Kpacked,
                         const float* b, float* out, int64_t ldo, int M, int N, int Npad, int K, int act, const int64_t* num_ims,
                         int rows_per_slide, float w_scale, float a_scale, hipStream_t stream) {
  PATHS_REQUIRE((a != nullptr) != (a_rows != nullptr), "gemm_add_nt_x6: exactly one of a / a_rows");
  PATHS_REQUIRE(a_add != nullptr && ld_add % 4 == 0 && (uintptr_t)a_add % 16 == 0, "gemm_add_nt_x6: a_add must be 16-byte aligned with ld_add %% 4 == 0");
  PATHS_REQUIRE(pow2(w_scale) && pow2(a_scale) && K == Kpacked && (Npad % 256 == 0 || Npad % 192 == 0),
                "gemm_add_nt_x6: power-of-two scales, whole-K image, Npad a multiple of 256 or of 192");
  X6Operands g{a, lda, K, a_rows, nullptr, 0, 0, a_add, ld_add, reinterpret_cast<const char*>(w_x6), group_stride(2, Kpacked), M, num_ims, rows_per_slide, a_scale};
  EpiBias e{b, out, ldo, N, act, nullptr, 0, nullptr, 0, 0, 1.0f / (w_scale * a_scale)};
  if (Npad % 256 != 0) {
    return a_rows ? launch_x6_np<2, 2, 3, 2, true, true>(g, Npad, e, stream, "gemm_add_nt_x6(rows, 192-wide tiles)")
                  : launch_x6_np<2, 2, 3, 2, true, false>(g, Npad, e, stream, "gemm_add_nt_x6(192-wide tiles)");
  }
  return a_rows ? launch_x6_np<2, 2, 4, 2, true, true>(g, Npad, e, stream, "gemm_add_nt_x6(rows)")
                : launch_x6_np<2, 2, 4, 2, true, false>(g, Npad, e, stream, "gemm_add_nt_x6");
}

int paths_gemm_add_nt_x6_h16(const float* a, int64_t lda, const int64_t* a_rows, const float* a_add, int64_t ld_add, const void* w_x6, int Kpacked,
                             const float* b, float* out, int64_t ldo, int M, int N, int Npad, int K, int act, const int64_t* num_ims,
                             int rows_per_slide, float w_scale, float a_scale, hipStream_t stream) {
  PATHS_REQUIRE(a == nullptr && a_rows != nullptr, "gemm_add_nt_x6_h16: fp16 rows are given as a_rows");
  PATHS_REQUIRE(a_add != nullptr && ld_add % 4 == 0 && (uintptr_t)a_add % 16 == 0, "gemm_add_nt_x6_h16: a_add must be 16-byte aligned with ld_add %% 4 == 0");
  PATHS_REQUIRE(pow2(w_scale) && pow2(a_scale) && K == Kpacked && (Npad % 256 == 0 || Npad % 192 == 0),
                "gemm_add_nt_x6_h16: power-of-two scales, whole-K image, Npad a multiple of 256 or of 192");
  X6Operands g{nullptr, lda, K, a_rows, nullptr, 0, 0, a_add, ld_add, reinterpret_cast<const char*>(w_x6), group_stride(2, Kpacked), M, num_ims, rows_per_slide, a_scale};
  EpiBias e{b, out, ldo, N, act, nullptr, 0, nullptr, 0, 0, 1.0f / (w_scale * a_scale)};
  if (Npad % 256 != 0) return launch_x6_np<2, 2, 3, 2, true, true, EpiBias, 1, true>(g, Npad, e, stream, "gemm_add_nt_x6_h16(rows, 192-wide tiles)");
  return launch_x6_np<2, 2, 4, 2, true, true, EpiBias, 1, true>(g, Npad, e, stream, "gemm_add_nt_x6_h16(rows)");
}

#endif

}
```

Baseline: 3792 slides/s.

## Stage two k16 sub-steps per LDS buffer in x6 GEMM for LSTM forms

Adds a KS template parameter so each LDS pipeline stage holds two k16 slices instead of one. This halves the number of barriers and stage switches per K loop, and gives more MFMAs in which to hide global loads and staging. It is enabled only for the row-pointer LSTM c and o GEMMs with PF=1 when the K window allows it; the PF=2 forms stay off behind a constexpr flag. The cost is double the LDS per stage, which can lower occupancy, plus longer unrolled code.

Measured after the change: 3796 slides/s, median of 4. Within noise of the previous version (+0.1%).

```diff
diff --git a/include/paths_hip.h b/include/paths_hip.h
--- a/include/paths_hip.h
+++ b/include/paths_hip.h
@@ -41,6 +41,7 @@
                           int skip_padding, paths_stream_t stream);
 
 int64_t paths_x6_packed_bytes(int Npad, int K, int planes);
+int paths_x6_k32_stages(int k_window, int K0, int pf);
 int paths_x6_pack_weights(const float* w, int64_t ldw, void* out, int N, int Npad, int K, int planes, float w_scale,
                           paths_stream_t stream);
 int paths_x6_pack_weights_t(const float* w, int64_t ldw, void* out, int N, int Npad, int K, int Kvalid, int planes, paths_stream_t stream);
diff --git a/paths_amd/_lib.py b/paths_amd/_lib.py
--- a/paths_amd/_lib.py
+++ b/paths_amd/_lib.py
@@ -129,7 +129,7 @@
 for _n in ("paths_lstm_cell_x6", "paths_importance_proj_x6", "paths_importance_qkv_x6", "paths_gemm_add_nt_x6", "paths_gather_rows",
            "paths_level0_batch", "paths_tissue_mask_absmax", "paths_synth_grid"):
     SIGNATURES[_n + "_h16"] = SIGNATURES[_n]
-_PLAIN = {"paths_gemm_tn_workspace": (C.c_int64, [_i32, _i32, _i32]), "paths_x6_packed_bytes": (C.c_int64, [_i32, _i32, _i32]), "paths_tlayer_h3_image_bytes": (C.c_int64, [_i32]), "paths_tlayer_ws_image_bytes": (C.c_int64, [_i32, _i32]), "paths_token0_ws_image_bytes": (C.c_int64, []), "paths_token0_ws_partials": (C.c_int64, [_i32, _i32]), "paths_token0_ws_image_bytes_d": (C.c_int64, [_i32]), "paths_token0_ws_partials_d": (C.c_int64, [_i32, _i32, _i32]), "paths_token0_ws_supported": (_i32, [_i32, _i32, _i32, _i32]), "paths_attention_x6_workspace": (C.c_int64, [_i32, _i32, _i32, _i32, _i32]), "paths_attention_fp8_workspace": (C.c_int64, [_i32, _i32, _i32, _i32]), "paths_attention_bwd_x6_workspace": (C.c_int64, [_i32, _i32, _i32, _i32]), "paths_attention_token0_workspace": (C.c_int64, [_i32, _i32, _i32]), "paths_token0_attention_workspace": (C.c_int64, [_i32, _i32, _i32, _i32]), "paths_attention_rollout_workspace": (C.c_int64, [_i32, _i32, _i32, _i32]), "paths_attention_h3_any_workspace": (C.c_int64, [_i32, _i32, _i32, _i32]), "paths_importance_proj_x6_workspace": (C.c_int64, [_i32]), "paths_last_error": (C.c_char_p, []), "paths_build_info": (C.c_char_p, []), "paths_abi_version": (_i32, []), "paths_stop_event_pending": (_i32, []), "paths_clear_stop_event": (_i32, []), "paths_adamw_chunk": (_i32, []), "paths_attention_wide_workspace": (C.c_int64, [_i32, _i32]), "paths_event_create": (_vp, []), "paths_stream_create_masked": (_vp, [_vp, _i32])}
+_PLAIN = {"paths_gemm_tn_workspace": (C.c_int64, [_i32, _i32, _i32]), "paths_x6_packed_bytes": (C.c_int64, [_i32, _i32, _i32]), "paths_x6_k32_stages": (_i32, [_i32, _i32, _i32]), "paths_tlayer_h3_image_bytes": (C.c_int64, [_i32]), "paths_tlayer_ws_image_bytes": (C.c_int64, [_i32, _i32]), "paths_token0_ws_image_bytes": (C.c_int64, []), "paths_token0_ws_partials": (C.c_int64, [_i32, _i32]), "paths_token0_ws_image_bytes_d": (C.c_int64, [_i32]), "paths_token0_ws_partials_d": (C.c_int64, [_i32, _i32, _i32]), "paths_token0_ws_supported": (_i32, [_i32, _i32, _i32, _i32]), "paths_attention_x6_workspace": (C.c_int64, [_i32, _i32, _i32, _i32, _i32]), "paths_attention_fp8_workspace": (C.c_int64, [_i32, _i32, _i32, _i32]), "paths_attention_bwd_x6_workspace": (C.c_int64, [_i32, _i32, _i32, _i32]), "paths_attention_token0_workspace": (C.c_int64, [_i32, _i32, _i32]), "paths_token0_attention_workspace": (C.c_int64, [_i32, _i32, _i32, _i32]), "paths_attention_rollout_workspace": (C.c_int64, [_i32, _i32, _i32, _i32]), "paths_attention_h3_any_workspace": (C.c_int64, [_i32, _i32, _i32, _i32]), "paths_importance_proj_x6_workspace": (C.c_int64, [_i32]), "paths_last_error": (C.c_char_p, []), "paths_build_info": (C.c_char_p, []), "paths_abi_version": (_i32, []), "paths_stop_event_pending": (_i32, []), "paths_clear_stop_event": (_i32, []), "paths_adamw_chunk": (_i32, []), "paths_attention_wide_workspace": (C.c_int64, [_i32, _i32]), "paths_event_create": (_vp, []), "paths_stream_create_masked": (_vp, [_vp, _i32])}
 
 ABI_VERSION = 3
 _lib: Optional[C.CDLL] = None
diff --git a/paths_amd/csrc/gemm_x6.hip b/paths_amd/csrc/gemm_x6.hip
--- a/paths_amd/csrc/gemm_x6.hip
+++ b/paths_amd/csrc/gemm_x6.hip
@@ -28,9 +28,10 @@
   int ksplit = 1;
 };
 
-template <int NP, int WTM, int WTN, int PF, bool ADD, bool ROWS, class Epi, int OCC = 1, bool A16 = false>
+template <int NP, int WTM, int WTN, int PF, bool ADD, bool ROWS, class Epi, int OCC = 1, bool A16 = false, int KS = 1>
 __global__ void __launch_bounds__(256) __attribute__((amdgpu_waves_per_eu(OCC, OCC)))
 gemm_x6_kernel(X6Operands g, Epi epi) {
+  static_assert(KS == 1 || KS == 2, "one or two k16 sub-steps per stage");
   static_assert(NP == 2 || NP == 3 || NP == 4, "two fp16 planes, three bf16 planes or two bf16 planes");
   static_assert(!A16 || (NP == 2 && ROWS), "fp16 A rows: two-plane fp16 split, row-pointer form");
   constexpr int PL = planes_of<NP>();
@@ -41,9 +42,10 @@
   constexpr int NPROD = NP == 3 ? 6 : A1P ? 2 : 3;
   constexpr int BM = WTM * 64, BN = WTN * 64;
   constexpr int SA = 2 * WTM, SB = 2 * WTN;
-  constexpr int STAGE = SA * SUBTA + SB * SUBT;
-  constexpr int NA = BM / 64;
-  constexpr int NPB = SB * PL, NB = (NPB + 3) / 4;
+  constexpr int STAGE1 = SA * SUBTA + SB * SUBT;
+  constexpr int STAGE = KS * STAGE1;
+  constexpr int NA1 = BM / 64, NA = KS * NA1;
+  constexpr int NPB = SB * PL, NB1 = (NPB + 3) / 4, NB = KS * NB1;
   static_assert(WTM % 2 == 0, "A fragment register slots alternate per accumulator row");
   extern __shared__ __attribute__((aligned(16))) char smem[];
   const int tid = threadIdx.x, lane = tid & 63, wave = __builtin_amdgcn_readfirstlane(tid >> 6), wm = wave >> 1, wn = wave & 1;
@@ -59,13 +61,13 @@
   if (block_all_padding(g.num_ims, g.rows_per_slide, m0, BM, g.M)) return;
 
   const int arow = tid >> 2, ac = tid & 3;
-  uint32_t aoff0[NA], aoff1[NA], aoffs[ADD ? NA : 1]; int awr[NA];
+  uint32_t aoff0[NA1], aoff1[NA1], aoffs[ADD ? NA1 : 1]; int awr[NA1];
   typedef const f32x4 __attribute__((address_space(1))) * gptr_f4;
   typedef const u32x2 __attribute__((address_space(1))) * gptr_h4;
-  gptr_f4 rowp[ROWS && !A16 ? NA : 1];
-  gptr_h4 rowh[A16 ? NA : 1];
-#pragma unroll
-  for (int p = 0; p < NA; ++p) {
+  gptr_f4 rowp[ROWS && !A16 ? NA1 : 1];
+  gptr_h4 rowh[A16 ? NA1 : 1];
+#pragma unroll
+  for (int p = 0; p < NA1; ++p) {
     const int row = p * 64 + arow;
     const int64_t grow = min(m0 + row, g.M - 1);
     aoff0[p] = ROWS ? 0u : (uint32_t)((grow * g.lda0 + 4 * ac) * 4);
@@ -79,17 +81,17 @@
   const int kofs = g.ksplit > 1 ? (int)blockIdx.z * K0w : 0;
   if (kofs != 0) {
 #pragma unroll
-    for (int p = 0; p < NA; ++p) {
+    for (int p = 0; p < NA1; ++p) {
       aoff0[p] += (uint32_t)kofs * 4u;
       if constexpr (A16) rowh[p] += kofs >> 2;
       else if constexpr (ROWS) rowp[p] += kofs >> 2;
       if constexpr (ADD) aoffs[p] += (uint32_t)kofs * 4u;
     }
   }
-  const int nk0 = K0w >> 4, nk = (K0w + g.K1) >> 4;
-  const char* bbase[NB]; int bwr[NB];
-#pragma unroll
-  for (int i = 0; i < NB; ++i) {
+  const int nk0 = K0w >> 4, nk = ((K0w + g.K1) >> 4) / KS;
+  const char* bbase[NB1]; int bwr[NB1];
+#pragma unroll
+  for (int i = 0; i < NB1; ++i) {
     int pc = wave + 4 * i;
     if (pc >= NPB) pc -= 4;
     const int sub = pc / PL, pl = pc % PL;
@@ -106,28 +108,30 @@
   const auto rsAdd = __builtin_amdgcn_make_buffer_rsrc(ADD ? const_cast<float*>(g.Aadd) : anyA, 0, 0xFFFFFFFFu, 0x00020000);
   const auto rsW = __builtin_amdgcn_make_buffer_rsrc(const_cast<char*>(g.Wt), 0, 0xFFFFFFFFu, 0x00020000);
   const int lane16 = lane * 16;
-  int bsoff[NB];
-#pragma unroll
-  for (int i = 0; i < NB; ++i) bsoff[i] = (int)(bbase[i] - g.Wt) + (kofs >> 4) * SUBT;
-  auto gload_a = [&](int set, int q, int kt) {
+  int bsoff[NB1];
+#pragma unroll
+  for (int i = 0; i < NB1; ++i) bsoff[i] = (int)(bbase[i] - g.Wt) + (kofs >> 4) * SUBT;
+  auto gload_a = [&](int set, int q, int st) {
+    const int p = q % NA1, kt = st * KS + q / NA1;
     const bool first = kt < nk0;
     const int soff = (first ? kt : kt - nk0) * 64;
     if constexpr (A16) {
-      sh[set][q] = rowh[q][kt * 4];
+      sh[set][q] = rowh[p][kt * 4];
     } else if constexpr (ROWS) {
-      sa[set][q] = rowp[q][kt * 4];
+      sa[set][q] = rowp[p][kt * 4];
     } else {
-      const u32x4 raw = first ? __builtin_amdgcn_raw_buffer_load_b128(rsA0, (int)aoff0[q], soff, 0)
-                              : __builtin_amdgcn_raw_buffer_load_b128(rsA1, (int)aoff1[q], soff, 0);
+      const u32x4 raw = first ? __builtin_amdgcn_raw_buffer_load_b128(rsA0, (int)aoff0[p], soff, 0)
+                              : __builtin_amdgcn_raw_buffer_load_b128(rsA1, (int)aoff1[p], soff, 0);
       sa[set][q] = __builtin_bit_cast(f32x4, raw);
     }
     if constexpr (ADD) {
-      sadd[set][q] = __builtin_bit_cast(f32x4, __builtin_amdgcn_raw_buffer_load_b128(rsAdd, (int)aoffs[q], kt * 64, 0));
+      sadd[set][q] = __builtin_bit_cast(f32x4, __builtin_amdgcn_raw_buffer_load_b128(rsAdd, (int)aoffs[p], kt * 64, 0));
     }
   };
-  auto gload_b = [&](int set, int q, int kt) {
-    sbr[set][q] = __builtin_amdgcn_raw_buffer_load_b128(rsW, lane16, bsoff[q] + kt * SUBT, 0);
+  auto gload_b = [&](int set, int q, int st) {
+    sbr[set][q] = __builtin_amdgcn_raw_buffer_load_b128(rsW, lane16, bsoff[q % NB1] + (st * KS + q / NB1) * SUBT, 0);
   };
+  auto awr_of = [&](int q) __attribute__((always_inline)) { return awr[q % NA1] + (q / NA1) * STAGE1; };
   constexpr int PRE = ADD ? (A16 ? 2 : 1) : 0;
   constexpr int NS = A1P ? 2 : (NP == 3 ? 12 : NP == 4 ? 7 : 5) + PRE;
   float tf[NA][2];
@@ -146,7 +150,7 @@
         asm("v_pk_mul_f16 %0, %1, %2" : "=v"(hi[q][0]) : "v"(sh[set][q][0]), "v"(s2));
         asm("v_pk_mul_f16 %0, %1, %2" : "=v"(hi[q][1]) : "v"(sh[set][q][1]), "v"(s2));
       }
-      if (st == 1) *reinterpret_cast<u32x2*>(smem + buf * STAGE + awr[q]) = u32x2{hi[q][0], hi[q][1]};
+      if (st == 1) *reinterpret_cast<u32x2*>(smem + buf * STAGE + awr_of(q)) = u32x2{hi[q][0], hi[q][1]};
     } else if constexpr (NP == 3) {
       if (st == 0) { hi[q][0] = pk_bf16(v[0], v[1]); hi[q][1] = pk_bf16(v[2], v[3]); }
       if (st == 1) { tf[q][0] = bf_lo(hi[q][0]); tf[q][1] = bf_hi(hi[q][0]); }
@@ -160,7 +164,7 @@
       if (st == 9) { v[2] -= tf[q][0]; v[3] -= tf[q][1]; }
       if (st == 10) { lo[q][0] = pk_bf16(v[0], v[1]); lo[q][1] = pk_bf16(v[2], v[3]); }
       if (st == 11) {
-        char* d = smem + buf * STAGE + awr[q];
+        char* d = smem + buf * STAGE + awr_of(q);
         *reinterpret_cast<u32x2*>(d) = u32x2{hi[q][0], hi[q][1]};
         *reinterpret_cast<u32x2*>(d + FRAG) = u32x2{mid[q][0], mid[q][1]};
         *reinterpret_cast<u32x2*>(d + 2 * FRAG) = u32x2{lo[q][0], lo[q][1]};
@@ -173,7 +177,7 @@
       if (st == 4) { v[2] -= tf[q][0]; v[3] -= tf[q][1]; }
       if (st == 5) { mid[q][0] = pk_bf16(v[0], v[1]); mid[q][1] = pk_bf16(v[2], v[3]); }
       if (st == 6) {
-        char* d = smem + buf * STAGE + awr[q];
+        char* d = smem + buf * STAGE + awr_of(q);
         *reinterpret_cast<u32x2*>(d) = u32x2{hi[q][0], hi[q][1]};
         *reinterpret_cast<u32x2*>(d + FRAG) = u32x2{mid[q][0], mid[q][1]};
       }
@@ -189,13 +193,13 @@
         asm("v_fma_mixhi_f16 %0, %1, -1.0, %2 op_sel:[1,0,0] op_sel_hi:[1,0,0]" : "+v"(lo[q][1]) : "v"(hi[q][1]), "v"(v[3]));
       }
       if (st == 4) {
-        char* d = smem + buf * STAGE + awr[q];
+        char* d = smem + buf * STAGE + awr_of(q);
         *reinterpret_cast<u32x2*>(d) = u32x2{hi[q][0], hi[q][1]};
         *reinterpret_cast<u32x2*>(d + FRAG) = u32x2{lo[q][0], lo[q][1]};
       }
     }
   };
-  auto swrite_b = [&](int set, int q, int buf) { *reinterpret_cast<u32x4*>(smem + buf * STAGE + bwr[q]) = sbr[set][q]; };
+  auto swrite_b = [&](int set, int q, int buf) { *reinterpret_cast<u32x4*>(smem + buf * STAGE + (q / NB1) * STAGE1 + bwr[q % NB1]) = sbr[set][q]; };
 
   f32x16 acc[WTM][WTN];
   epi.template init<WTM, WTN>(acc, m0 + wm * WTM * 32, n0 + wn * WTN * 32, lane, g.M);
@@ -203,8 +207,8 @@
   const char* sA = smem + (wm * WTM) * SUBTA + lane * 16;
   const char* sB = A1P ? smem + SA * SUBTA + (wn * WTN) * SUBT + lane * 16 : smem + (SA + wn * WTN) * SUBT + lane * 16;
   u32x4 fa[2][PLA], fb[2][WTN][PL];
-  auto read_a = [&](int buf, int i, int slot, int p) { fa[slot][p] = *reinterpret_cast<const u32x4*>(sA + buf * STAGE + i * SUBTA + p * FRAG); };
-  auto read_b = [&](int buf, int j, int slot, int p) { fb[slot][j][p] = *reinterpret_cast<const u32x4*>(sB + buf * STAGE + j * SUBT + p * FRAG); };
+  auto read_a = [&](int buf, int u, int i, int slot, int p) { fa[slot][p] = *reinterpret_cast<const u32x4*>(sA + buf * STAGE + u * STAGE1 + i * SUBTA + p * FRAG); };
+  auto read_b = [&](int buf, int u, int j, int slot, int p) { fb[slot][j][p] = *reinterpret_cast<const u32x4*>(sB + buf * STAGE + u * STAGE1 + j * SUBT + p * FRAG); };
   constexpr int RG = WTN * NPROD;
   auto one_mfma = [&](int gq, int sb) __attribute__((always_inline)) {
     const int i = gq / RG, j = (gq % RG) / NPROD, t = gq % NPROD, sl = i & 1;
@@ -223,15 +227,18 @@
     }
   };
   constexpr int AG = (WTM - 1) * RG;
+  constexpr int SG = WTM * RG;
+  constexpr int PRE_S = KS * AG;
+  constexpr int TOT_S = KS * SG - (KS - 1) * RG;
   constexpr auto fits = [](int spg) constexpr {
-    return PF == 1 ? ((NS + spg - 1) / spg) * NA + NB <= AG : (NS * NA + spg - 1) / spg + NB <= AG;
+    return PF == 1 ? ((NS + spg - 1) / spg) * NA + NB <= PRE_S : (NS * NA + spg - 1) / spg + NB <= PRE_S;
   };
   constexpr int SPG = fits(1) ? 1 : fits(2) ? 2 : fits(3) ? 3 : 4;
   static_assert(fits(SPG), "staging does not fit before the barrier");
   constexpr int GPC = (NS + SPG - 1) / SPG;
   constexpr int GA2 = (NS * NA + SPG - 1) / SPG;
   constexpr int TS = PF == 1 ? GPC * NA + NB : GA2 + NB + NA + NB;
-  static_assert(TS <= WTM * RG, "staging does not fit in a stage");
+  static_assert(TS <= TOT_S, "staging does not fit in a stage");
   constexpr int AR0 = RG / 2;
   auto staging_slot = [&](auto sc, int kt, auto bufc, auto m1c, auto m2c) __attribute__((always_inline)) {
     constexpr int s = decltype(sc)::value, buf = decltype(bufc)::value;
@@ -268,29 +275,38 @@
     }
   };
   auto stage_body = [&](int kt, auto bufc, auto m1c, auto m2c) __attribute__((always_inline)) {
-    constexpr int buf = decltype(bufc)::value, sb = buf;
-    constexpr bool more1 = decltype(m1c)::value, more2 = decltype(m2c)::value;
-    constexpr int set = PF == 2 ? (buf ^ 1) : 0;
-    static_for<0, AG>([&](auto gc) __attribute__((always_inline)) {
-      constexpr int gq = decltype(gc)::value, i = gq / RG, gr = gq % RG;
-      one_mfma(gq, sb);
-      if constexpr (gr >= AR0 && gr < AR0 + PLA) read_a(buf, i + 1, (i + 1) & 1, gr - AR0);
-      staging_slot(std::integral_constant<int, gq>{}, kt, bufc, m1c, m2c);
+    constexpr int buf = decltype(bufc)::value;
+    constexpr bool more1 = decltype(m1c)::value;
+    static_for<0, KS * SG - RG>([&](auto gc) __attribute__((always_inline)) {
+      constexpr int gq = decltype(gc)::value, u = gq / SG, w = gq % SG, i = w / RG, gr = w % RG;
+      constexpr int sb = KS == 1 ? buf : (u & 1);
+      one_mfma(w, sb);
+      if constexpr (i < WTM - 1) {
+        if constexpr (gr >= AR0 && gr < AR0 + PLA) read_a(buf, u, i + 1, (i + 1) & 1, gr - AR0);
+        staging_slot(std::integral_constant<int, gq - u * RG>{}, kt, bufc, m1c, m2c);
+      } else {
+        static_for<2 * gr, 2 * gr + 2>([&](auto fc) __attribute__((always_inline)) {
+          constexpr int f = decltype(fc)::value;
+          if constexpr (f < PLA) read_a(buf, u + 1, 0, 0, f);
+          else if constexpr (f < PLA + PL * WTN) read_b(buf, u + 1, (f - PLA) / PL, sb ^ 1, (f - PLA) % PL);
+        });
+      }
       __builtin_amdgcn_sched_barrier(0);
     });
     __syncthreads();
     __builtin_amdgcn_sched_barrier(0);
-    static_for<AG, WTM * RG>([&](auto gc) __attribute__((always_inline)) {
-      constexpr int gq = decltype(gc)::value, gr = gq % RG;
-      one_mfma(gq, sb);
+    static_for<KS * SG - RG, KS * SG>([&](auto gc) __attribute__((always_inline)) {
+      constexpr int gq = decltype(gc)::value, w = gq % SG, gr = w % RG;
+      constexpr int sb = KS == 1 ? buf : ((KS - 1) & 1);
+      one_mfma(w, sb);
       if constexpr (more1) {
         static_for<2 * gr, 2 * gr + 2>([&](auto fc) __attribute__((always_inline)) {
           constexpr int f = decltype(fc)::value;
-          if constexpr (f < PLA) read_a(buf ^ 1, 0, 0, f);
-          else if constexpr (f < PLA + PL * WTN) read_b(buf ^ 1, (f - PLA) / PL, sb ^ 1, (f - PLA) % PL);
+          if constexpr (f < PLA) read_a(buf ^ 1, 0, 0, 0, f);
+          else if constexpr (f < PLA + PL * WTN) read_b(buf ^ 1, 0, (f - PLA) / PL, sb ^ 1, (f - PLA) % PL);
         });
       }
-      staging_slot(std::integral_constant<int, gq>{}, kt, bufc, m1c, m2c);
+      staging_slot(std::integral_constant<int, gq - (KS - 1) * RG>{}, kt, bufc, m1c, m2c);
       __builtin_amdgcn_sched_barrier(0);
     });
   };
@@ -318,11 +334,11 @@
   }
   __syncthreads();
 #pragma unroll
-  for (int p = 0; p < PLA; ++p) read_a(0, 0, 0, p);
+  for (int p = 0; p < PLA; ++p) read_a(0, 0, 0, 0, p);
 #pragma unroll
   for (int j = 0; j < WTN; ++j)
 #pragma unroll
-    for (int p = 0; p < PL; ++p) read_b(0, j, 0, p);
+    for (int p = 0; p < PL; ++p) read_b(0, 0, j, 0, p);
   for (int kt = 0; kt < nk - 2 * PF; kt += 2) {
     __builtin_amdgcn_sched_barrier(0);
     stage_body(kt, I0, T, T);
@@ -335,7 +351,9 @@
   stage_body(nk - 2, I0, T, F);
   stage_body(nk - 1, I1, F, F);
   __syncthreads();
-  epi.template run<WTM, WTN, 2, 2>(acc, m0 + wm * WTM * 32, n0 + wn * WTN * 32, lane, wm, wn, g.M, reinterpret_cast<float*>(smem));
+  int lane_e = lane;
+  if constexpr (KS == 2) lane_e = (int)__builtin_amdgcn_mbcnt_hi(~0u, __builtin_amdgcn_mbcnt_lo(~0u, 0u));
+  epi.template run<WTM, WTN, 2, 2>(acc, m0 + wm * WTM * 32, n0 + wn * WTN * 32, lane_e, wm, wn, g.M, reinterpret_cast<float*>(smem));
 }
 
 template <int NP>
@@ -384,25 +402,36 @@
   if constexpr (NP == 3) *reinterpret_cast<u16x8*>(o + FRAG) = u16x8{l[0], l[1], l[2], l[3], l[4], l[5], l[6], l[7]};
 }
 
-template <int NP, int WTM, int WTN, int PF, bool ADD, bool ROWS, class Epi, int OCC = 1, bool A16 = false>
+inline bool k32_window_ok(int kwin, int K0, int pf) { return kwin % 64 == 0 && kwin >= 64 * pf && K0 % 32 == 0; }
+constexpr bool K32_PF2_FORMS = false;
+
+template <int NP, int WTM, int WTN, int PF, bool ADD, bool ROWS, class Epi, int OCC = 1, bool A16 = false, bool K32 = false>
 int launch_x6_np(const X6Operands& g, int Npad, const Epi& epi, hipStream_t stream, const char* name) {
   constexpr int BM = WTM * 64, BN = WTN * 64;
-  constexpr size_t lds = 2ull * (2 * WTM * ((A16 && !ADD) ? FRAG : subt<NP>()) + 2 * WTN * subt<NP>());
+  constexpr size_t lds1 = 2ull * (2 * WTM * ((A16 && !ADD) ? FRAG : subt<NP>()) + 2 * WTN * subt<NP>());
   const int K = g.K0 + g.K1;
   PATHS_REQUIRE(g.M > 0, "%s: M must be > 0", name);
-  PATHS_REQUIRE(g.K0 > 0 && g.K0 % 16 == 0 && g.K1 % 16 == 0 && K % 32 == 0 && K >= 128, "%s: K panels (%d,%d): multiples of 16, total a multiple of 32, >= 128", name, g.K0, g.K1);
+  PATHS_REQUIRE(g.K0 > 0 && g.K0 % 16 == 0 && g.K1 % 16 == 0 && K % 32 == 0 && K >= 64, "%s: K panels (%d,%d): multiples of 16, total a multiple of 32, >= 64", name, g.K0, g.K1);
   PATHS_REQUIRE(Npad % BN == 0, "%s: packed N (%d) must be a multiple of %d", name, Npad, BN);
   PATHS_REQUIRE(g.lda0 % 4 == 0 && g.lda1 % 4 == 0, "%s: leading dims must be multiples of 4 floats", name);
   PATHS_REQUIRE(((uintptr_t)g.A0 % 16 == 0) && ((uintptr_t)g.A1 % 16 == 0) && ((uintptr_t)g.Wt % 16 == 0), "%s: operands must be 16-byte aligned", name);
   PATHS_REQUIRE(ROWS == (g.A0rows != nullptr) && (!ROWS || g.K1 == 0), "%s: row-pointer form is single-panel", name);
   PATHS_REQUIRE((int64_t)g.M * (g.lda0 > g.lda1 ? (g.lda0 > g.ldadd ? g.lda0 : g.ldadd) : (g.lda1 > g.ldadd ? g.lda1 : g.ldadd)) * 4 < (int64_t)1 << 32, "%s: A panel larger than 4 GiB", name);
-  auto kern = gemm_x6_kernel<NP, WTM, WTN, PF, ADD, ROWS, Epi, OCC, A16>;
-  PATHS_LDS_OPT_IN(kern, lds, name);
   PATHS_REQUIRE(g.ksplit == 1 || (g.ksplit > 1 && g.K1 == 0 && g.K0 % (32 * g.ksplit) == 0 && g.K0 / g.ksplit >= 128), "%s: split-K needs a single panel and k windows that are multiples of 32, >= 128", name);
-  dim3 grid(Npad / BN, (g.M + BM - 1) / BM, g.ksplit);
-  hipLaunchKernelGGL(kern, grid, dim3(256), lds, stream, g, epi);
-  PATHS_LAUNCH_CHECK(name);
-  return PATHS_OK;
+  const dim3 grid(Npad / BN, (g.M + BM - 1) / BM, g.ksplit);
+  auto go = [&](auto ksc) -> int {
+    constexpr int KS = decltype(ksc)::value;
+    constexpr size_t lds = KS * lds1;
+    auto kern = gemm_x6_kernel<NP, WTM, WTN, PF, ADD, ROWS, Epi, OCC, A16, KS>;
+    PATHS_LDS_OPT_IN(kern, lds, name);
+    hipLaunchKernelGGL(kern, grid, dim3(256), lds, stream, g, epi);
+    PATHS_LAUNCH_CHECK(name);
+    return PATHS_OK;
+  };
+  if constexpr (K32) {
+    if (k32_window_ok(g.ksplit > 1 ? g.K0 / g.ksplit : K, g.K0, PF)) return go(std::integral_constant<int, 2>{});
+  }
+  return go(std::integral_constant<int, 1>{});
 }
 
 struct EpiRaw {
@@ -456,10 +485,16 @@
   epi.template run<1, 4, 2, 2>(acc, row0, col0, lane, wm, wn, M, reinterpret_cast<float*>(smem));
 }
 
+template <class Epi, int WTM, int WTN, int PF, bool ADD>
+constexpr bool k32_rows_form() {
+  return !ADD && ((std::is_same<Epi, EpiLstmC>::value && WTM == 4 && WTN == 3 && PF == 1) || (std::is_same<Epi, EpiLstmORaw>::value && WTM == 4 && WTN == 4 && PF == 1) ||
+                  (K32_PF2_FORMS && std::is_same<Epi, EpiBias>::value && WTM == 2 && WTN == 4 && PF == 2));
+}
+
 template <int WTM, int WTN, int PF, bool ADD, class Epi>
 int launch_x6(int planes, const X6Operands& g, int Npad, const Epi& epi, hipStream_t stream, const char* name) {
   if (g.A0rows != nullptr) {
-    if (planes == 2) return launch_x6_np<2, WTM, WTN, PF, ADD, true>(g, Npad, epi, stream, name);
+    if (planes == 2) return launch_x6_np<2, WTM, WTN, PF, ADD, true, Epi, 1, false, k32_rows_form<Epi, WTM, WTN, PF, ADD>()>(g, Npad, epi, stream, name);
     return paths_set_error(PATHS_EUNSUPPORTED, "%s: row pointers need planes = 2", name);
   }
   if constexpr (std::is_same<Epi, EpiBias>::value && !ADD) {
@@ -484,6 +519,8 @@
 
 #if PATHS_X6_PART == 0 || PATHS_X6_PART == 1
 int64_t paths_x6_packed_bytes(int Npad, int K, int planes) { return (int64_t)Npad * K * 2 * plane_count(planes); }
+
+int paths_x6_k32_stages(int k_window, int K0, int pf) { return (pf == 1 || K32_PF2_FORMS) && k32_window_ok(k_window, K0, pf) ? 1 : 0; }
 
 int paths_x6_pack_weights(const float* w, int64_t ldw, void* out, int N, int Npad, int K, int planes, float w_scale, hipStream_t stream) {
   PATHS_REQUIRE(N > 0 && Npad >= N && Npad % 32 == 0 && K % 16 == 0, "x6_pack_weights: bad shape N=%d Npad=%d K=%d", N, Npad, K);
@@ -539,7 +576,7 @@
     int rc;
     if constexpr (A16) {
       rc = small_m ? launch_x6_np<2, 2, 3, 2, false, true, decltype(e), 1, true>(g, 3 * Hc, e, stream, "lstm_cell_x6_h16(c, 128-row tiles)")
-                   : launch_x6_np<2, 4, 3, 1, false, true, decltype(e), 1, true>(g, 3 * Hc, e, stream, "lstm_cell_x6_h16(c)");
+                   : launch_x6_np<2, 4, 3, 1, false, true, decltype(e), 1, true, true>(g, 3 * Hc, e, stream, "lstm_cell_x6_h16(c)");
     } else if (small_m) rc = x_rows ? launch_x6_np<2, 2, 3, 2, false, true>(g, 3 * Hc, e, stream, "lstm_cell_x6(c, 128-row tiles)")
                              : launch_x6_np<2, 2, 3, 2, false, false>(g, 3 * Hc, e, stream, "lstm_cell_x6(c, 128-row tiles)");
     else rc = launch_x6<4, 3, 1, false>(planes, g, 3 * Hc, e, stream, "lstm_cell_x6(c)");
@@ -554,7 +591,7 @@
       EpiLstmORaw e{b_gates + 3 * Hc, ws_o, D, D, hp, (int64_t)3 * Hc + D, hp_row, 3 * Hc, sg};
       if constexpr (A16) {
         rc = small_m ? launch_x6_np<2, 2, 4, 2, false, true, decltype(e), 1, true>(go, D, e, stream, "lstm_cell_x6_h16(o, raw, 128-row tiles)")
-                     : launch_x6_np<2, 4, 4, 1, false, true, decltype(e), 1, true>(go, D, e, stream, "lstm_cell_x6_h16(o, raw)");
+                     : launch_x6_np<2, 4, 4, 1, false, true, decltype(e), 1, true, true>(go, D, e, stream, "lstm_cell_x6_h16(o, raw)");
       } else if (small_m) rc = x_rows ? launch_x6_np<2, 2, 4, 2, false, true>(go, D, e, stream, "lstm_cell_x6(o, raw, 128-row tiles)")
                                : launch_x6_np<2, 2, 4, 2, false, false>(go, D, e, stream, "lstm_cell_x6(o, raw, 128-row tiles)");
       else rc = launch_x6<4, 4, 1, false>(planes, go, D, e, stream, "lstm_cell_x6(o, raw)");
@@ -650,12 +687,12 @@
         if constexpr (A16) {
           X6Operands gs = g; gs.ksplit = 2;
           EpiRaw raw{splitk_ws, zstride, 8};
-          rc = launch_x6_np<2, 2, 4, 2, true, true, EpiRaw, 1, true>(gs, 256, raw, stream, "importance_proj_x6_h16(split-k)");
+          rc = launch_x6_np<2, 2, 4, 2, true, true, EpiRaw, 1, true, K32_PF2_FORMS>(gs, 256, raw, stream, "importance_proj_x6_h16(split-k)");
         } else {
           X6Operands gs = g; gs.ksplit = 2;
           EpiRaw raw{splitk_ws, zstride, 8};
           rc = y_add == nullptr ? launch_x6_np<2, 2, 4, 2, false, false>(gs, 256, raw, stream, "importance_proj_x6(split-k, stored y)")
-               : y_rows ? launch_x6_np<2, 2, 4, 2, true, true>(gs, 256, raw, stream, "importance_proj_x6(split-k)")
+               : y_rows ? launch_x6_np<2, 2, 4, 2, true, true, EpiRaw, 1, false, K32_PF2_FORMS>(gs, 256, raw, stream, "importance_proj_x6(split-k)")
                         : launch_x6_np<2, 2, 4, 2, true, false>(gs, 256, raw, stream, "importance_proj_x6(split-k)");
         }
         if (rc != PATHS_OK) return rc;
@@ -730,8 +767,8 @@
     g.ksplit = 2;
     EpiRaw raw{splitk_ws, zstride, 8};
     int rc;
-    if constexpr (A16) rc = launch_x6_np<2, 2, 4, 2, true, true, EpiRaw, 1, true>(g, 256, raw, stream, "importance_qkv_x6_h16(split-k)");
-    else rc = y_rows ? launch_x6_np<2, 2, 4, 2, true, true>(g, 256, raw, stream, "importance_qkv_x6(split-k)")
+    if constexpr (A16) rc = launch_x6_np<2, 2, 4, 2, true, true, EpiRaw, 1, true, K32_PF2_FORMS>(g, 256, raw, stream, "importance_qkv_x6_h16(split-k)");
+    else rc = y_rows ? launch_x6_np<2, 2, 4, 2, true, true, EpiRaw, 1, false, K32_PF2_FORMS>(g, 256, raw, stream, "importance_qkv_x6(split-k)")
                      : launch_x6_np<2, 2, 4, 2, true, false>(g, 256, raw, stream, "importance_qkv_x6(split-k)");
     if (rc != PATHS_OK) return rc;
   }
```
